# shg8/3DGS.cpp

Hardware: NVIDIA H100
Metric: frames/sec (higher is better)
Workload: dtype f32

## Files before the change

3dgs.cpp_b200/csrc/gsb_api.cu:

```cuda
#include <math.h>
#include <stdio.h>
#include <stdlib.h>
#include <string.h>

#include <algorithm>
#include <new>
#include <thread>
#include <vector>

#include "gsb_ctx.cuh"

using namespace gsb;

namespace {
thread_local std::string g_create_error;
}

namespace gsb {

int fail(gsb_ctx* c, int code, const char* what, cudaError_t e) {
    if (c) {
        c->err = what;
        if (e != cudaSuccess) {
            c->err += ": ";
            c->err += cudaGetErrorString(e);
        }
    }
    return code;
}

void drop_graphs(gsb_ctx* ctx) {
    for (auto& g : ctx->graphs) {
        if (g.exec) cudaGraphExecDestroy(g.exec);
        g = MiddleGraph{};
    }
}

template <typename T>
static int grow_zeroed(gsb_ctx* ctx, DevArray<T>& a, uint64_t count, const char* name) {
    if (count <= a.count) return GSB_OK;
    const char* step = "cudaMalloc";
    cudaError_t e = a.grow(count);
    if (e == cudaSuccess) {
        step = "cudaMemsetAsync";
        e = cudaMemsetAsync(a, 0, count * sizeof(T), ctx->stream);
    }
    if (e == cudaSuccess) {
        step = "cudaStreamSynchronize";
        e = cudaStreamSynchronize(ctx->stream);
    }
    if (e == cudaSuccess) return GSB_OK;
    a.reset();
    return fail(ctx, e == cudaErrorMemoryAllocation ? GSB_ERR_OOM : GSB_ERR_CUDA, (std::string(step) + " of " + name).c_str(), e);
}

int ensure_sort_status(gsb_ctx* ctx, uint64_t items) {
    const uint32_t tiles = (uint32_t)((items + sort_tile_items() - 1) / sort_tile_items());
    if ((uint64_t)tiles * 256 <= ctx->sort_status.count) return GSB_OK;
    ctx->alloc_gen++;
    return grow_zeroed(ctx, ctx->sort_status, (uint64_t)tiles * 256, "ctx->sort_status");
}

int ensure_arena(gsb_ctx* ctx, uint64_t capacity) {
    if (capacity <= ctx->capacity) return GSB_OK;
    if (capacity >= (1ull << 30)) return fail(ctx, GSB_ERR_OVERFLOW, "instance arena limited to 2^30 - 1 entries");
    ctx->capacity = 0;
    ctx->alloc_gen++;
    ctx->frame.recorded = false;
    CK(ctx->keys[0].grow(capacity + 16));
    CK(ctx->keys[1].grow(capacity + 16));
    CK(ctx->vals[0].grow(capacity + 16));
    CK(ctx->vals[1].grow(capacity + 16));
    int rc = ensure_sort_status(ctx, std::max<uint64_t>(capacity, ctx->n));
    if (rc != GSB_OK) return rc;
    ctx->capacity = capacity;
    return GSB_OK;
}

uint32_t bits_for(uint32_t count) {
    uint32_t b = 0;
    while (b < 32 && (1ull << b) < count) b++;
    return b;
}

uint32_t quantise_hint(uint64_t hint) {
    uint64_t q = 4096;
    while (q < hint && q < (1ull << 31)) q <<= 1;
    return (uint32_t)q;
}

size_t bytes_per_pixel(int fmt) { return fmt == GSB_FORMAT_RGBA32F ? 16 : 4; }

static void take_hints(gsb_ctx* ctx) {
    ctx->frame.pending = false;
    ctx->m_hint = ctx->ctl_host->num_instances;
    ctx->nv_hint = ctx->ctl_host->num_visible;
}

int wait_frame(gsb_ctx* ctx) {
    if (ctx->frame.pending) {
        CK(cudaEventSynchronize(ctx->ev_done));
        take_hints(ctx);
    }
    return GSB_OK;
}

void poll_frame(gsb_ctx* ctx) {
    if (ctx->frame.pending && cudaEventQuery(ctx->ev_done) == cudaSuccess) take_hints(ctx);
}

int regrow_after_overflow(gsb_ctx* ctx, cudaStream_t stream) {
    if (!ctx->ctl_host->overflow) return GSB_OK;
    const uint64_t want = ctx->ctl_host->instances_total + ctx->ctl_host->instances_total / 4 + 4096;
    int rc = ensure_arena(ctx, want);
    if (rc != GSB_OK) return rc;
    CK(cudaMemsetAsync(&ctx->ctl->overflow_sticky, 0, sizeof(uint32_t), stream));
    ctx->regrow_count++;
    return GSB_OK;
}

static __global__ void k_frame_init(Control* ctl, uint32_t* __restrict__ project_status, uint32_t project_chunks,
                                    unsigned long long* __restrict__ emit_status, uint32_t emit_chunks, uint2* __restrict__ ranges,
                                    uint32_t num_tiles, uint32_t* __restrict__ route_status, uint32_t route_words) {
    const uint32_t i = blockIdx.x * blockDim.x + threadIdx.x, stride = gridDim.x * blockDim.x;
    uint32_t* w = reinterpret_cast<uint32_t*>(ctl);
    for (uint32_t k = i; k < sizeof(Control) / 4; k += stride) {
        if (k == offsetof(Control, overflow_sticky) / 4) continue;
        if (k == offsetof(Control, epoch) / 4) w[k] += 16u;
        else w[k] = 0u;
    }
    for (uint32_t k = i; k < project_chunks; k += stride) project_status[k] = 0u;
    for (uint32_t k = i; k < emit_chunks; k += stride) emit_status[k] = 0ull;
    for (uint32_t k = i; k < num_tiles; k += stride) ranges[k] = make_uint2(0xffffffffu, 0xffffffffu);
    for (uint32_t k = i; k < route_words; k += stride) route_status[k] = 0u;
}

cudaError_t launch_frame_init(Control* ctl, uint32_t* project_status, uint32_t project_chunks, unsigned long long* emit_status,
                              uint32_t emit_chunks, uint2* ranges, uint32_t num_tiles, cudaStream_t s, uint32_t* route_status,
                              uint32_t route_words) {
    const uint32_t work = std::max<uint32_t>(std::max(std::max(std::max(project_chunks, emit_chunks), num_tiles), route_words),
                                             (uint32_t)(sizeof(Control) / 4));
    const uint32_t blocks = std::min<uint32_t>((work + 255) / 256, 132u * 4u);
    k_frame_init<<<blocks, 256, 0, s>>>(ctl, project_status, project_chunks, emit_status, emit_chunks, ranges, num_tiles, route_status,
                                        route_words);
    return cudaGetLastError();
}

int enqueue_middle(gsb_ctx* ctx, const FramePlan& fp, const Survivors& sv, cudaStream_t stream, bool events) {
    SortParams sa;
    sa.keys[0] = sv.dkeys[0];
    sa.keys[1] = sv.dkeys[1];
    sa.vals[0] = sv.dvals[0];
    sa.vals[1] = sv.dvals[1];
    sa.d_m = &ctx->ctl->num_visible;
    sa.m_hint = fp.nv_q;
    sa.key_bits = 32;
    sa.status = ctx->sort_status;
    sa.status_tiles = (uint32_t)(ctx->sort_status.count / 256);
    sa.d_epoch = &ctx->ctl->epoch;
    sa.sc = &ctx->ctl->sort_depth;
    sa.num_sms = ctx->num_sms;
    sa.discard_sorted_keys = true;
    uint32_t depth_passes = 0;
    CK(launch_sort(sa, &depth_passes, stream));
    const int fin_a = depth_passes & 1;
    if (events) CK(cudaEventRecord(ctx->ev[2], stream));

    EmitParams ep{};
    ep.sorted_cid = sv.dvals[fin_a];
    ep.nv_hint = fp.nv_q;
    ep.tiles_x = fp.bins_x;
    ep.coarse_shift = fp.cs;
    ep.keys = ctx->keys[0];
    ep.vals = ctx->vals[0];
    ep.capacity = (uint32_t)ctx->capacity;
    ep.status = sv.emit_status;
    ep.ctl = ctx->ctl;
    ep.num_sms = ctx->num_sms;
    ep.recs = sv.recs;
    ep.cull = (ctx->tile_cull >= 1 && fp.cs == 0) ? 1 : 0;
    ep.dbg_offsets = ctx->debug ? ctx->dbg_offsets.p : nullptr;
    CK(launch_emit(ep, stream));
    if (events) CK(cudaEventRecord(ctx->ev[3], stream));

    if (ctx->debug) {
        CK(cudaStreamSynchronize(stream));
        uint32_t m = 0;
        CK(cudaMemcpy(&m, &ctx->ctl->num_instances, sizeof m, cudaMemcpyDeviceToHost));
        if (ctx->dbg_keys_unsorted) CK(cudaDeviceSynchronize());
        CK(ctx->dbg_keys_unsorted.grow(m));
        CK(ctx->dbg_vals_unsorted.grow(m));
        CK(cudaMemcpyAsync(ctx->dbg_keys_unsorted, ctx->keys[0], (size_t)m * 4, cudaMemcpyDeviceToDevice, stream));
        CK(cudaMemcpyAsync(ctx->dbg_vals_unsorted, ctx->vals[0], (size_t)m * 4, cudaMemcpyDeviceToDevice, stream));
    }

    SortParams sp;
    sp.keys[0] = ctx->keys[0];
    sp.keys[1] = ctx->keys[1];
    sp.vals[0] = ctx->vals[0];
    sp.vals[1] = ctx->vals[1];
    sp.d_m = &ctx->ctl->num_instances;
    sp.m_hint = fp.m_q;
    sp.key_bits = bits_for(fp.bins);
    sp.status = ctx->sort_status;
    sp.status_tiles = (uint32_t)(ctx->sort_status.count / 256);
    sp.d_epoch = &ctx->ctl->epoch;
    sp.epoch_base = 4;
    sp.sc = &ctx->ctl->sort_tile;
    sp.num_sms = ctx->num_sms;
    sp.events = events ? ctx->ev_sort : nullptr;
    sp.ranges = ctx->ranges;
    sp.discard_sorted_keys = !ctx->debug && fp.cs == 0;
    sp.range_key_mask = fp.cs ? 0xffffu : 0u;
    uint32_t passes = 0;
    CK(launch_sort(sp, &passes, stream));
    if (events) CK(cudaEventRecord(ctx->ev[4], stream));
    if (passes == 0) CK(launch_ranges_single_tile(sp.d_m, ctx->ranges, stream));
    if (events) CK(cudaEventRecord(ctx->ev[5], stream));
    if (depth_passes != fp.depth_passes || passes != fp.passes) return fail(ctx, GSB_ERR_CUDA, "internal: pass count mismatch");
    return GSB_OK;
}

int launch_middle_graph(gsb_ctx* ctx, const FramePlan& fp, const Survivors& sv, cudaStream_t stream) {
    MiddleKey key;
    key.tiles_x = fp.tiles_x;
    key.num_tiles = fp.T;
    key.nv_q = fp.nv_q;
    key.m_q = fp.m_q;
    key.cull = (uint32_t)ctx->tile_cull;
    key.cs = fp.cs;
    key.alloc_gen = ctx->alloc_gen;
    key.sv = sv;
    MiddleGraph* slot = nullptr;
    for (auto& g : ctx->graphs)
        if (g.exec && g.key == key) slot = &g;
    if (!slot) {
        slot = &ctx->graphs[0];
        for (auto& g : ctx->graphs)
            if (!g.exec || (slot->exec && g.last_use < slot->last_use)) slot = &g;
        if (slot->exec) cudaGraphExecDestroy(slot->exec);
        *slot = MiddleGraph{};
        cudaGraph_t graph = nullptr;
        CK(cudaStreamBeginCapture(ctx->stream, cudaStreamCaptureModeThreadLocal));
        int rc = enqueue_middle(ctx, fp, sv, ctx->stream, false);
        cudaError_t e = cudaStreamEndCapture(ctx->stream, &graph);
        if (rc != GSB_OK) {
            if (graph) cudaGraphDestroy(graph);
            return rc;
        }
        if (e != cudaSuccess) return fail(ctx, GSB_ERR_CUDA, "cudaStreamEndCapture", e);
        e = cudaGraphInstantiate(&slot->exec, graph, 0);
        cudaGraphDestroy(graph);
        if (e != cudaSuccess) {
            slot->exec = nullptr;
            return fail(ctx, GSB_ERR_CUDA, "cudaGraphInstantiate", e);
        }
        slot->key = key;
    }
    slot->last_use = ++ctx->graph_clock;
    CK(cudaGraphLaunch(slot->exec, stream));
    return GSB_OK;
}

int ensure_ranges(gsb_ctx* ctx, uint32_t W, uint32_t H) {
    const uint32_t T = ((W + GSB_TILE - 1) / GSB_TILE) * ((H + GSB_TILE - 1) / GSB_TILE);
    if (T > ctx->ranges.count) {
        ctx->alloc_gen++;
        CK(ctx->ranges.grow(T));
    }
    return GSB_OK;
}

int plan_frame(gsb_ctx* ctx, const gsb_uniforms* ubo, uint32_t rb, uint32_t re, cudaStream_t stream, FramePlan* out) {
    FramePlan fp{};
    fp.W = ubo->width;
    fp.H = ubo->height;
    fp.tiles_x = (fp.W + GSB_TILE - 1) / GSB_TILE;
    fp.tiles_y = (fp.H + GSB_TILE - 1) / GSB_TILE;
    fp.T = fp.tiles_x * fp.tiles_y;
    fp.rb = rb;
    fp.re = re;
    {
        int rc = ensure_ranges(ctx, fp.W, fp.H);
        if (rc != GSB_OK) return rc;
    }
    const uint32_t n = (uint32_t)ctx->n;
    fp.nv_q = std::min<uint32_t>(quantise_hint(ctx->nv_hint ? ctx->nv_hint : n), quantise_hint(n));
    fp.m_q = quantise_hint(ctx->m_hint ? ctx->m_hint : std::min<uint64_t>(ctx->capacity, 4u * 1024 * 1024));
    fp.cs = (ctx->tile_cull == 2 && !ctx->debug && !ctx->backward) ? ctx->coarse_shift : 0u;
    fp.bins_x = (fp.tiles_x + (1u << fp.cs) - 1) >> fp.cs;
    fp.bins = fp.bins_x * ((fp.tiles_y + (1u << fp.cs) - 1) >> fp.cs);
    if (fp.cs && fp.bins > 65536u) {
        fp.cs = 0;
        fp.bins_x = fp.tiles_x;
        fp.bins = fp.T;
    }
    fp.depth_passes = 4;
    fp.passes = (bits_for(fp.bins) + 7) / 8;
    fp.fin = (int)(fp.passes & 1);
    if (++ctx->frames_since_epoch_clear >= (1u << 27)) {
        CK(cudaMemsetAsync(ctx->sort_status, 0, ctx->sort_status.count * sizeof(unsigned long long), stream));
        CK(cudaMemsetAsync(&ctx->ctl->epoch, 0, sizeof(uint32_t), stream));
        ctx->frames_since_epoch_clear = 0;
    }
    *out = fp;
    return GSB_OK;
}

ProjectParams project_params(const gsb_ctx* ctx, const gsb_uniforms& ubo, uint32_t rb, uint32_t re) {
    ProjectParams pp{};
    pp.pos_op = ctx->pos_op;
    pp.cov_a = ctx->cov_a;
    pp.cov_b = ctx->cov_b;
    pp.sh = ctx->sh;
    pp.sh_half = ctx->scene_sh_half ? 1 : 0;
    pp.n = (uint32_t)ctx->n;
    pp.ubo = ubo;
    pp.tile_row_begin = rb;
    pp.tile_row_end = re;
    pp.recs = ctx->recs;
    pp.dkeys = ctx->dkeys[0];
    pp.dvals = ctx->dvals[0];
    pp.status = ctx->project_status;
    pp.ctl = ctx->ctl;
    pp.dbg_tiles = ctx->dbg_tiles;
    pp.dbg_aabb = ctx->dbg_aabb;
    return pp;
}

static int enqueue_front(gsb_ctx* ctx, const gsb_uniforms* ubo, uint32_t rb, uint32_t re, const Survivors& sv, cudaStream_t stream,
                         FramePlan* out) {
    FramePlan fp{};
    int rc = plan_frame(ctx, ubo, rb, re, stream, &fp);
    if (rc != GSB_OK) return rc;
    const uint32_t chunks = (uint32_t)((ctx->n + 255) / 256);
    const bool timers = ctx->timers;
    CK(launch_frame_init(ctx->ctl, ctx->project_status, std::max(chunks, 1u), ctx->emit_status, std::max(chunks, 1u), ctx->ranges, fp.T, stream));
    if (timers) CK(cudaEventRecord(ctx->ev[0], stream));

    CK(launch_project(project_params(ctx, *ubo, rb, re), ctx->debug, ctx->antialiased, stream));
    if (timers) CK(cudaEventRecord(ctx->ev[1], stream));

    if (ctx->use_graph && !timers && !ctx->debug) rc = launch_middle_graph(ctx, fp, sv, stream);
    else rc = enqueue_middle(ctx, fp, sv, stream, timers);
    if (rc != GSB_OK) return rc;
    *out = fp;
    return GSB_OK;
}

int enqueue_blend(gsb_ctx* ctx, const FramePlan& fp, const Survivors& sv, uint32_t b0, uint32_t b1, void* band_out, size_t pitch,
                  int fmt, cudaStream_t stream, void* const* peer_frames, int num_peer_frames) {
    BlendParams bp{};
    bp.recs = sv.recs;
    bp.vals = ctx->vals[fp.fin];
    bp.keys = ctx->keys[fp.fin];
    bp.ranges = ctx->ranges;
    bp.width = fp.W;
    bp.height = fp.H;
    bp.tiles_x = fp.tiles_x;
    bp.coarse_shift = fp.cs;
    bp.bins_x = fp.bins_x;
    bp.tile_row_begin = b0;
    bp.tile_row_end = b1;
    bp.out = static_cast<unsigned char*>(band_out) + (size_t)(b0 - fp.rb) * GSB_TILE * pitch;
    bp.out_first_row = b0 * GSB_TILE;
    bp.num_peers = num_peer_frames;
    for (int k = 0; k < num_peer_frames && k < GSB_MAX_SHARDS; k++) bp.peer_frames[k] = peer_frames[k];
    if (num_peer_frames > 0) bp.out_first_row = 0;
    bp.row_pitch_bytes = pitch;
    bp.format = fmt;
    bp.mode = ctx->mode;
    bp.stats = ctx->debug ? 2 : (ctx->timers ? 1 : 0);
    bp.ctl = ctx->ctl;
    bp.record = (ctx->backward && fp.cs == 0 && num_peer_frames == 0) ? ctx->bw_record.p : nullptr;
    for (int c = 0; c < 3; c++) bp.background[c] = ctx->background[c];
    CK(launch_blend(bp, stream));
    return GSB_OK;
}

int enqueue_tail(gsb_ctx* ctx, const FramePlan& fp, const gsb_uniforms& ubo, cudaStream_t stream) {
    if (ctx->timers) CK(cudaEventRecord(ctx->ev[6], stream));
    CK(cudaMemcpyAsync(ctx->ctl_host, ctx->ctl, offsetof(Control, sort_depth), cudaMemcpyDeviceToHost, stream));
    CK(cudaEventRecord(ctx->ev_done, stream));
    LastFrame& f = ctx->frame;
    f.plan = fp;
    f.ubo = ubo;
    f.mode = ctx->mode;
    f.antialiased = ctx->antialiased;
    for (int c = 0; c < 3; c++) f.background[c] = ctx->background[c];
    f.scene_gen = ctx->scene_gen;
    f.pending = true;
    f.exists = true;
    f.debug = ctx->debug;
    f.timers = ctx->timers;
    f.recorded = ctx->backward && fp.cs == 0;
    f.band = !(fp.rb == 0 && fp.re == fp.tiles_y);
    return GSB_OK;
}

static int enqueue_frame(gsb_ctx* ctx, const gsb_uniforms* ubo, uint32_t rb, uint32_t re, void* out_dev, size_t pitch, int fmt,
                  cudaStream_t stream) {
    ctx->frame.recorded = false;
    if (ctx->backward) CK(ctx->bw_record.grow((size_t)ubo->width * ubo->height));
    const Survivors sv{ctx->recs, {ctx->dkeys[0], ctx->dkeys[1]}, {ctx->dvals[0], ctx->dvals[1]}, ctx->emit_status};
    FramePlan fp{};
    int rc = enqueue_front(ctx, ubo, rb, re, sv, stream, &fp);
    if (rc != GSB_OK) return rc;
    rc = enqueue_blend(ctx, fp, sv, rb, re, out_dev, pitch, fmt, stream);
    if (rc != GSB_OK) return rc;
    return enqueue_tail(ctx, fp, *ubo, stream);
}

int check_image(gsb_ctx* ctx, const gsb_uniforms* ubo, int fmt) {
    if (fmt < GSB_FORMAT_RGBA32F || fmt > GSB_FORMAT_BGRA8) return fail(ctx, GSB_ERR_INVALID, "bad format");
    const uint32_t W = ubo->width, H = ubo->height;
    if (W == 0 || H == 0 || W > 16u * 65535u || H > 16u * 65535u) return fail(ctx, GSB_ERR_INVALID, "bad image size");
    return GSB_OK;
}

int check_render_args(gsb_ctx* ctx, const gsb_uniforms* ubo, uint32_t& rb, uint32_t& re, const void* out, size_t& pitch,
                      int fmt) {
    if (!ctx) return GSB_ERR_INVALID;
    if (!ubo || !out) return fail(ctx, GSB_ERR_INVALID, "null argument");
    if (!ctx->pos_op) return fail(ctx, GSB_ERR_NO_SCENE, "no scene uploaded");
    const int rc = check_image(ctx, ubo, fmt);
    if (rc != GSB_OK) return rc;
    const uint32_t W = ubo->width, H = ubo->height;
    const uint32_t tiles_y = (H + GSB_TILE - 1) / GSB_TILE;
    if (re > tiles_y) re = tiles_y;
    if (rb >= re) return fail(ctx, GSB_ERR_INVALID, "empty tile-row band");
    const size_t tight = (size_t)W * bytes_per_pixel(fmt);
    if (pitch == 0) pitch = tight;
    if (pitch < tight || (pitch % (fmt == GSB_FORMAT_RGBA32F ? 16 : 4)) != 0) return fail(ctx, GSB_ERR_INVALID, "bad row pitch");
    return GSB_OK;
}

}

extern "C" {

int gsb_abi_version(void) { return GSB_ABI_VERSION; }

int gsb_device_count(void) {
    int n = 0;
    if (cudaGetDeviceCount(&n) != cudaSuccess) {
        cudaGetLastError();
        return 0;
    }
    return n;
}

const char* gsb_last_error(const gsb_ctx* ctx) { return ctx ? ctx->err.c_str() : g_create_error.c_str(); }

int gsb_create(int device, gsb_ctx** out) {
    if (!out) return GSB_ERR_INVALID;
    *out = nullptr;
    int count = 0;
    cudaError_t e = cudaGetDeviceCount(&count);
    if (e != cudaSuccess || count <= 0 || device < 0 || device >= count) {
        cudaGetLastError();
        g_create_error = "no usable CUDA device (libgsb200 has no CPU path)";
        if (e != cudaSuccess) g_create_error += std::string(": ") + cudaGetErrorString(e);
        return GSB_ERR_NO_DEVICE;
    }
    gsb_ctx* ctx = new (std::nothrow) gsb_ctx();
    if (!ctx) return GSB_ERR_OOM;
    ctx->device = device;
    auto bail = [&](const char* what, cudaError_t err) {
        g_create_error = std::string(what) + ": " + cudaGetErrorString(err);
        gsb_destroy(ctx);
        return GSB_ERR_CUDA;
    };
    if ((e = cudaSetDevice(device)) != cudaSuccess) return bail("cudaSetDevice", e);
    cudaDeviceProp prop;
    if ((e = cudaGetDeviceProperties(&prop, device)) != cudaSuccess) return bail("cudaGetDeviceProperties", e);
    cudaFuncAttributes fa;
    if (prop.major != 9 || prop.minor != 0 || cudaFuncGetAttributes(&fa, k_frame_init) != cudaSuccess) {
        cudaGetLastError();
        g_create_error = "libgsb200 is built for sm_90a (H100, compute capability 9.0) only; device is sm_" +
                         std::to_string(prop.major) + std::to_string(prop.minor);
        gsb_destroy(ctx);
        return GSB_ERR_NO_DEVICE;
    }
    ctx->num_sms = prop.multiProcessorCount;
    if (const char* v = getenv("GSB_HOST_DIRECT")) ctx->host_direct = atoi(v) != 0;
    if (const char* v = getenv("GSB_COARSE_SHIFT")) ctx->coarse_shift = (uint32_t)std::min(2, std::max(1, atoi(v)));
    if ((e = sort_prepare()) != cudaSuccess) return bail("sort_prepare", e);
    if ((e = cudaStreamCreateWithFlags(&ctx->stream, cudaStreamNonBlocking)) != cudaSuccess) return bail("cudaStreamCreate", e);
    if ((e = dev_alloc(&ctx->ctl, 1)) != cudaSuccess) return bail("cudaMalloc", e);
    if ((e = cudaMemset(ctx->ctl, 0, sizeof(Control))) != cudaSuccess) return bail("cudaMemset", e);
    if ((e = cudaDeviceSynchronize()) != cudaSuccess) return bail("cudaDeviceSynchronize", e);
    if ((e = cudaMallocHost(reinterpret_cast<void**>(&ctx->ctl_host), sizeof(Control))) != cudaSuccess) return bail("cudaMallocHost", e);
    memset(ctx->ctl_host, 0, sizeof(Control));
    for (auto& ev : ctx->ev)
        if ((e = cudaEventCreate(&ev)) != cudaSuccess) return bail("cudaEventCreate", e);
    for (auto& ev : ctx->ev_sort)
        if ((e = cudaEventCreate(&ev)) != cudaSuccess) return bail("cudaEventCreate", e);
    if ((e = cudaEventCreateWithFlags(&ctx->ev_done, cudaEventDisableTiming)) != cudaSuccess) return bail("cudaEventCreate", e);
    *out = ctx;
    return GSB_OK;
}

void gsb_destroy(gsb_ctx* ctx) {
    if (!ctx) return;
    cudaSetDevice(ctx->device);
    if (ctx->stream) cudaStreamSynchronize(ctx->stream);
    cudaDeviceSynchronize();
    drop_graphs(ctx);
    shard_destroy(ctx);
    if (ctx->ctl) cudaFree(ctx->ctl);
    if (ctx->ctl_host) cudaFreeHost(ctx->ctl_host);
    for (auto& ev : ctx->ev)
        if (ev) cudaEventDestroy(ev);
    for (auto& ev : ctx->ev_sort)
        if (ev) cudaEventDestroy(ev);
    if (ctx->ev_done) cudaEventDestroy(ctx->ev_done);
    if (ctx->stream) cudaStreamDestroy(ctx->stream);
    delete ctx;
}

int gsb_scene_upload(gsb_ctx* ctx, const float* vertices, uint64_t n, gsb_memory mem) {
    if (!ctx) return GSB_ERR_INVALID;
    if (n && !vertices) return fail(ctx, GSB_ERR_INVALID, "null vertices");
    if (n >= (1ull << 30)) return fail(ctx, GSB_ERR_INVALID, "scene limited to 2^30 - 1 Gaussians");
    CK(cudaSetDevice(ctx->device));
    CK(cudaStreamSynchronize(ctx->stream));
    if (ctx->pos_op) CK(cudaDeviceSynchronize());
    ctx->frame.pending = ctx->frame.exists = false;
    ctx->n = 0;
    ctx->alloc_gen++;
    ctx->scene_gen++;
    drop_graphs(ctx);
    CK(ctx->pos_op.grow(n));
    CK(ctx->cov_a.grow(n));
    CK(ctx->cov_b.grow(n));
    ctx->scene_sh_half = ctx->sh_half;
    CK(ctx->sh.grow(n * (ctx->scene_sh_half ? 24 : 48)));
    CK(ctx->recs.grow(n * GSB_REC_F4));
    CK(ctx->dkeys[0].grow(n));
    CK(ctx->dkeys[1].grow(n));
    CK(ctx->dvals[0].grow(n));
    CK(ctx->dvals[1].grow(n));
    CK(ctx->project_status.grow((n + 255) / 256));
    CK(ctx->emit_status.grow((n + 255) / 256));
    if (ctx->debug) {
        CK(ctx->dbg_tiles.grow(n));
        CK(ctx->dbg_aabb.grow(n));
        CK(ctx->dbg_offsets.grow(n));
    }
    if (mem == GSB_MEM_DEVICE) {
        const uint64_t chunk = std::min<uint64_t>(std::max<uint64_t>(n, 1), 1u << 20);
        for (uint64_t off = 0; off < n; off += chunk) {
            const uint64_t cnt = std::min(chunk, n - off);
            cudaError_t e = launch_cov3d(vertices + off * 60, cnt, off, ctx->pos_op, ctx->cov_a, ctx->cov_b, ctx->sh, 1.0f, ctx->stream, ctx->scene_sh_half);
            if (e != cudaSuccess) return fail(ctx, GSB_ERR_CUDA, "cov3d precompute", e);
        }
        CK(cudaStreamSynchronize(ctx->stream));
    } else if (n) {
        cudaPointerAttributes pa{};
        const bool caller_pinned = cudaPointerGetAttributes(&pa, vertices) == cudaSuccess && pa.type == cudaMemoryTypeHost;
        cudaGetLastError();
        const uint64_t chunk = std::min<uint64_t>(n, 1u << 18);
        float* dev_stage[2] = {nullptr, nullptr};
        float* pin_stage[2] = {nullptr, nullptr};
        cudaEvent_t slot_free[2] = {nullptr, nullptr};
        cudaError_t e = cudaSuccess;
        for (int k = 0; k < 2 && e == cudaSuccess; k++) {
            e = dev_alloc(&dev_stage[k], chunk * 60);
            if (e == cudaSuccess && !caller_pinned) e = cudaMallocHost(reinterpret_cast<void**>(&pin_stage[k]), chunk * 60 * sizeof(float));
            if (e == cudaSuccess) e = cudaEventCreateWithFlags(&slot_free[k], cudaEventDisableTiming);
        }
        const unsigned hw = std::max(1u, std::min(std::thread::hardware_concurrency(), 8u));
        uint64_t idx = 0;
        for (uint64_t off = 0; off < n && e == cudaSuccess; off += chunk, idx++) {
            const int k = (int)(idx & 1);
            const uint64_t cnt = std::min(chunk, n - off);
            const float* src = vertices + off * 60;
            if (idx >= 2) e = cudaEventSynchronize(slot_free[k]);
            if (e != cudaSuccess) break;
            if (!caller_pinned) {
                const size_t bytes = cnt * 60 * sizeof(float);
                const unsigned nt = bytes >= (8u << 20) ? hw : 1u;
                std::vector<std::thread> pool;
                const size_t per = (bytes / nt + 63) & ~size_t(63);
                for (unsigned t = 1; t < nt; t++) {
                    const size_t b = std::min(bytes, t * per), en = std::min(bytes, b + per);
                    if (b < en) pool.emplace_back([=] { memcpy(reinterpret_cast<char*>(pin_stage[k]) + b, reinterpret_cast<const char*>(src) + b, en - b); });
                }
                memcpy(pin_stage[k], src, std::min(bytes, per));
                for (auto& th : pool) th.join();
                src = pin_stage[k];
            }
            e = cudaMemcpyAsync(dev_stage[k], src, cnt * 60 * sizeof(float), cudaMemcpyHostToDevice, ctx->stream);
            if (e == cudaSuccess) e = launch_cov3d(dev_stage[k], cnt, off, ctx->pos_op, ctx->cov_a, ctx->cov_b, ctx->sh, 1.0f, ctx->stream, ctx->scene_sh_half);
            if (e == cudaSuccess) e = cudaEventRecord(slot_free[k], ctx->stream);
        }
        if (e == cudaSuccess) e = cudaStreamSynchronize(ctx->stream);
        else cudaStreamSynchronize(ctx->stream);
        for (int k = 0; k < 2; k++) {
            if (dev_stage[k]) cudaFree(dev_stage[k]);
            if (pin_stage[k]) cudaFreeHost(pin_stage[k]);
            if (slot_free[k]) cudaEventDestroy(slot_free[k]);
        }
        if (e != cudaSuccess) return fail(ctx, e == cudaErrorMemoryAllocation ? GSB_ERR_OOM : GSB_ERR_CUDA, "scene upload", e);
    }
    ctx->n = n;
    ctx->m_hint = 0;
    ctx->nv_hint = 0;
    {
        int rc = ensure_sort_status(ctx, std::max<uint64_t>(n, ctx->capacity));
        if (rc != GSB_OK) return rc;
    }
    if (ctx->capacity == 0) {
        int rc = ensure_arena(ctx, std::max<uint64_t>(n, 1024));
        if (rc != GSB_OK) return rc;
    }
    return GSB_OK;
}

uint64_t gsb_scene_size(const gsb_ctx* ctx) { return ctx ? ctx->n : 0; }

int gsb_set_mode(gsb_ctx* ctx, gsb_mode mode) {
    if (!ctx || (mode != GSB_MODE_EXACT && mode != GSB_MODE_FAST)) return GSB_ERR_INVALID;
    ctx->mode = mode;
    return GSB_OK;
}

int gsb_set_sh_storage(gsb_ctx* ctx, int half_precision) {
    if (!ctx) return GSB_ERR_INVALID;
    ctx->sh_half = half_precision != 0;
    return GSB_OK;
}

int gsb_set_debug(gsb_ctx* ctx, int debug) {
    if (!ctx) return GSB_ERR_INVALID;
    CK(cudaSetDevice(ctx->device));
    ctx->debug = debug != 0;
    if (ctx->debug && ctx->n) {
        CK(ctx->dbg_tiles.grow(ctx->n));
        CK(ctx->dbg_aabb.grow(ctx->n));
        CK(ctx->dbg_offsets.grow(ctx->n));
    }
    return GSB_OK;
}

int gsb_set_graph(gsb_ctx* ctx, int enabled) {
    if (!ctx) return GSB_ERR_INVALID;
    ctx->use_graph = enabled != 0;
    return GSB_OK;
}

int gsb_host_alloc(void** out, size_t bytes) {
    if (!out) return GSB_ERR_INVALID;
    *out = nullptr;
    cudaError_t e = cudaMallocHost(out, bytes ? bytes : 1);
    if (e != cudaSuccess) {
        cudaGetLastError();
        g_create_error = std::string("cudaMallocHost: ") + cudaGetErrorString(e);
        return e == cudaErrorMemoryAllocation ? GSB_ERR_OOM : GSB_ERR_CUDA;
    }
    return GSB_OK;
}

void gsb_host_free(void* p) {
    if (p) cudaFreeHost(p);
}

int gsb_set_tile_cull(gsb_ctx* ctx, int level) {
    if (!ctx || level < 0 || level > 2) return GSB_ERR_INVALID;
    ctx->tile_cull = level;
    return GSB_OK;
}

int gsb_set_timers(gsb_ctx* ctx, int enabled) {
    if (!ctx) return GSB_ERR_INVALID;
    ctx->timers = enabled != 0;
    return GSB_OK;
}

int gsb_reserve_instances(gsb_ctx* ctx, uint64_t capacity) {
    if (!ctx) return GSB_ERR_INVALID;
    CK(cudaSetDevice(ctx->device));
    int rc = wait_frame(ctx);
    if (rc != GSB_OK) return rc;
    return ensure_arena(ctx, capacity);
}

int gsb_render_async(gsb_ctx* ctx, const gsb_uniforms* ubo, uint32_t rb, uint32_t re, void* out_device, size_t pitch,
                     gsb_format fmt, void* stream) {
    int rc = check_render_args(ctx, ubo, rb, re, out_device, pitch, fmt);
    if (rc != GSB_OK) return rc;
    CK(cudaSetDevice(ctx->device));
    poll_frame(ctx);
    return enqueue_frame(ctx, ubo, rb, re, out_device, pitch, fmt, stream_or_own(ctx, stream));
}

int gsb_render(gsb_ctx* ctx, const gsb_uniforms* ubo, uint32_t rb, uint32_t re, void* out, size_t pitch, gsb_memory out_mem,
               gsb_format fmt, void* stream) {
    int rc = check_render_args(ctx, ubo, rb, re, out, pitch, fmt);
    if (rc != GSB_OK) return rc;
    CK(cudaSetDevice(ctx->device));
    cudaStream_t s = stream_or_own(ctx, stream);
    const uint32_t H = ubo->height;
    const uint32_t rows = std::min(H, re * GSB_TILE) - rb * GSB_TILE;
    const size_t tight = (size_t)ubo->width * bytes_per_pixel(fmt);

    void* dev_out = out;
    size_t dev_pitch = pitch;
    bool staged = false;
    if (out_mem == GSB_MEM_HOST) {
        cudaPointerAttributes pa{};
        const bool pinned = ctx->host_direct && cudaPointerGetAttributes(&pa, out) == cudaSuccess &&
                            pa.type == cudaMemoryTypeHost && pa.devicePointer != nullptr;
        cudaGetLastError();
        if (pinned) {
            dev_out = pa.devicePointer;
        } else {
            CK(ctx->fb.grow(tight * rows));
            dev_out = ctx->fb;
            dev_pitch = tight;
            staged = true;
        }
    }
    for (int attempt = 0;; attempt++) {
        rc = enqueue_frame(ctx, ubo, rb, re, dev_out, dev_pitch, fmt, s);
        if (rc != GSB_OK) return rc;
        rc = wait_frame(ctx);
        if (rc != GSB_OK) return rc;
        if (!ctx->ctl_host->overflow) break;
        if (attempt >= 3) return fail(ctx, GSB_ERR_OVERFLOW, "instance arena overflow persists after regrow");
        rc = regrow_after_overflow(ctx, s);
        if (rc != GSB_OK) return rc;
    }
    if (staged) {
        CK(cudaMemcpy2DAsync(out, pitch, dev_out, dev_pitch, tight, rows, cudaMemcpyDeviceToHost, s));
        CK(cudaStreamSynchronize(s));
    }
    return GSB_OK;
}

int gsb_get_stats(gsb_ctx* ctx, gsb_stats* out) {
    if (!ctx || !out) return GSB_ERR_INVALID;
    memset(out, 0, sizeof *out);
    if (!ctx->frame.exists) return fail(ctx, GSB_ERR_INVALID, "no frame rendered yet");
    CK(cudaSetDevice(ctx->device));
    const int rc = wait_frame(ctx);
    if (rc != GSB_OK) return rc;
    const Control* c = ctx->ctl_host;
    out->num_gaussians = ctx->n;
    out->num_visible = c->num_visible;
    out->num_instances = c->instances_total;
    out->num_instances_aabb = c->candidates_total;
    out->blend_consumed = c->blend_consumed;
    out->blend_warp_visits = c->blend_walked;
    out->blend_pixel_hits = c->blend_hits;
    out->blend_staged = c->blend_staged;
    out->instance_capacity = ctx->capacity;
    out->sort_passes = ctx->frame.plan.passes;
    out->sort_depth_passes = ctx->frame.plan.depth_passes;
    out->regrow_count = ctx->regrow_count;
    if (ctx->frame.timers) {
        float ms = 0.f;
        CK(cudaEventElapsedTime(&ms, ctx->ev[0], ctx->ev[1]));
        out->preprocess_ms = ms;
        CK(cudaEventElapsedTime(&ms, ctx->ev[1], ctx->ev[2]));
        out->sort_depth_ms = ms;
        CK(cudaEventElapsedTime(&ms, ctx->ev[2], ctx->ev[3]));
        out->preprocess_sort_ms = ms;
        CK(cudaEventElapsedTime(&ms, ctx->ev[3], ctx->ev[4]));
        out->sort_tile_ms = ms;
        out->sort_ms = out->sort_depth_ms + out->sort_tile_ms;
        if (ctx->frame.plan.passes) {
            CK(cudaEventElapsedTime(&ms, ctx->ev[3], ctx->ev_sort[0]));
            out->sort_hist_ms = ms;
            for (uint32_t p = 0; p < ctx->frame.plan.passes && p < 8; p++) {
                CK(cudaEventElapsedTime(&ms, ctx->ev_sort[p], ctx->ev_sort[p + 1]));
                out->sort_pass_ms[p] = ms;
            }
        }
        CK(cudaEventElapsedTime(&ms, ctx->ev[4], ctx->ev[5]));
        out->tile_boundary_ms = ms;
        CK(cudaEventElapsedTime(&ms, ctx->ev[5], ctx->ev[6]));
        out->render_ms = ms;
        CK(cudaEventElapsedTime(&ms, ctx->ev[0], ctx->ev[6]));
        out->frame_ms = ms;
        if (ctx->shard) {
            CK(cudaEventElapsedTime(&ms, ctx->ev[5], ctx->ev[7]));
            out->shard_blend_ms = ms;
            CK(cudaEventElapsedTime(&ms, ctx->ev[7], ctx->ev[6]));
            out->shard_wait_ms = ms;
        }
    }
    if (c->overflow || c->overflow_sticky) {
        CK(cudaMemsetAsync(&ctx->ctl->overflow_sticky, 0, sizeof(uint32_t), ctx->stream));
        CK(cudaStreamSynchronize(ctx->stream));
        ctx->ctl_host->overflow_sticky = 0;
        return fail(ctx, GSB_ERR_OVERFLOW, c->overflow ? "last frame overflowed the instance arena (gsb_render regrows; gsb_render_async does not)"
                                                       : "an earlier gsb_render_async frame overflowed the instance arena (its image is incomplete)");
    }
    return GSB_OK;
}

int gsb_set_backward(gsb_ctx* ctx, int enabled) {
    if (!ctx) return GSB_ERR_INVALID;
    if (ctx->shard) return fail(ctx, GSB_ERR_INVALID, "gsb_set_backward: sharded contexts have no backward pass");
    CK(cudaSetDevice(ctx->device));
    ctx->backward = enabled != 0;
    if (!ctx->backward) {
        CK(cudaStreamSynchronize(ctx->stream));
        ctx->bw_record.reset();
        ctx->frame.recorded = false;
        ctx->bw_det = {};
    }
    return GSB_OK;
}

int gsb_set_antialiased(gsb_ctx* ctx, int enabled) {
    if (!ctx) return GSB_ERR_INVALID;
    if (ctx->shard) return fail(ctx, GSB_ERR_INVALID, "gsb_set_antialiased: sharded contexts have no anti-aliased mode");
    ctx->antialiased = enabled != 0;
    return GSB_OK;
}

int gsb_set_background(gsb_ctx* ctx, const float* rgb) {
    if (!ctx) return GSB_ERR_INVALID;
    const float v[3] = {rgb ? rgb[0] : 0.0f, rgb ? rgb[1] : 0.0f, rgb ? rgb[2] : 0.0f};
    for (float x : v)
        if (!isfinite(x)) return fail(ctx, GSB_ERR_INVALID, "gsb_set_background: the colour must be finite");
    for (int c = 0; c < 3; c++) ctx->background[c] = v[c];
    return GSB_OK;
}

int gsb_set_backward_deterministic(gsb_ctx* ctx, int enabled) {
    if (!ctx) return GSB_ERR_INVALID;
    if (ctx->shard) return fail(ctx, GSB_ERR_INVALID, "gsb_set_backward_deterministic: sharded contexts have no backward pass");
    ctx->bw_deterministic = enabled != 0;
    return GSB_OK;
}

static int ensure_det_buffers(gsb_ctx* ctx, uint64_t n) {
    DetBuffers& d = ctx->bw_det;
    const uint64_t cap = ctx->capacity;
    CK(d.slots.grow(cap * 11));
    CK(d.keys[0].grow(cap));
    CK(d.keys[1].grow(cap));
    CK(d.pos[0].grow(cap));
    CK(d.pos[1].grow(cap));
    const uint32_t tiles = (uint32_t)((cap + sort_tile_items() - 1) / sort_tile_items());
    CK(d.status.grow((uint64_t)std::max<uint32_t>(tiles, 1) * 256));
    CK(d.sc.grow(1));
    if (n > d.runs.count) CK(d.runs.grow(n));
    return GSB_OK;
}

static int check_recorded_frame(gsb_ctx* ctx, int no_frame, const char* fn) {
    const LastFrame& f = ctx->frame;
    auto bad = [&](int code, const char* what) { return fail(ctx, code, (std::string(fn) + ": " + what).c_str()); };
    if (f.scene_gen == 0) return bad(no_frame, "no frame rendered yet");
    if (f.scene_gen != ctx->scene_gen) return bad(GSB_ERR_INVALID, "the scene was uploaded or stepped after the last frame");
    if (!f.recorded) return bad(GSB_ERR_INVALID, "the last frame was rendered with gsb_set_backward off, or the arena grew since");
    if (f.band) return bad(GSB_ERR_INVALID, "the last frame was a band of tile rows, not the whole frame");
    const int rc = wait_frame(ctx);
    if (rc != GSB_OK) return rc;
    if (ctx->ctl_host->overflow) return bad(GSB_ERR_INVALID, "the last frame overflowed the instance arena (its lists are incomplete)");
    return GSB_OK;
}

static int render_backward(gsb_ctx* ctx, const char* fn, bool args_ok, const float* vertices, const float* grad_image, size_t pitch,
                           float* grad_vertices, gsb_uniforms* grad_ubo, float* density, void* stream) {
    if (!ctx) return GSB_ERR_INVALID;
    auto msg = [&](const char* what) { return std::string(fn) + ": " + what; };
    if (ctx->shard) return fail(ctx, GSB_ERR_INVALID, msg("sharded contexts have no backward pass").c_str());
    if (!ctx->pos_op) return fail(ctx, GSB_ERR_NO_SCENE, msg("no scene uploaded").c_str());
    CK(cudaSetDevice(ctx->device));
    int rc = check_recorded_frame(ctx, GSB_ERR_NO_SCENE, fn);
    if (rc != GSB_OK) return rc;
    if (ctx->scene_sh_half) return fail(ctx, GSB_ERR_INVALID, msg("fp16 SH storage has no backward pass").c_str());
    if (!args_ok) return fail(ctx, GSB_ERR_INVALID, msg("null argument").c_str());
    const LastFrame& f = ctx->frame;
    const size_t tight = (size_t)f.ubo.width * sizeof(float4);
    if (pitch == 0) pitch = tight;
    if (pitch < tight || pitch % sizeof(float4) != 0) return fail(ctx, GSB_ERR_INVALID, msg("bad row pitch").c_str());
    const uint64_t n = ctx->n;
    rc = grow_zeroed(ctx, ctx->bw_scratch, n * 9, "ctx->bw_scratch");
    if (rc != GSB_OK) return rc;
    if (density) {
        rc = grow_zeroed(ctx, ctx->bw_abs, n * 2, "ctx->bw_abs");
        if (rc != GSB_OK) return rc;
    }
    if (grad_ubo)
        CK(ctx->bw_cam_partials.grow((uint64_t)ctx->num_sms * 4 * GSB_UBO_WORDS));
    const bool det = ctx->bw_deterministic;
    if (det) {
        rc = ensure_det_buffers(ctx, n);
        if (rc != GSB_OK) return rc;
    }
    cudaStream_t s = stream_or_own(ctx, stream);
    if (grad_vertices) CK(cudaMemsetAsync(grad_vertices, 0, (size_t)n * 60 * sizeof(float), s));
    if (n == 0) {
        if (grad_ubo) CK(cudaMemsetAsync(grad_ubo, 0, sizeof(gsb_uniforms), s));
        return GSB_OK;
    }
    BackwardParams bp{};
    bp.recs = ctx->recs;
    bp.vals = ctx->vals[f.plan.fin];
    bp.ranges = ctx->ranges;
    bp.record = ctx->bw_record;
    bp.ctl = ctx->ctl;
    bp.width = f.ubo.width;
    bp.height = f.ubo.height;
    bp.tiles_x = f.plan.tiles_x;
    bp.num_tiles = f.plan.T;
    bp.mode = f.mode;
    bp.ubo = f.ubo;
    bp.vertices = vertices;
    bp.cov_a = ctx->cov_a;
    bp.cov_b = ctx->cov_b;
    bp.grad_image = grad_image;
    bp.row_pitch_bytes = pitch;
    bp.scratch = ctx->bw_scratch;
    bp.grad_vertices = grad_vertices;
    bp.num_sms = ctx->num_sms;
    bp.cam_partials = grad_ubo ? ctx->bw_cam_partials.p : nullptr;
    bp.grad_ubo = grad_ubo;
    bp.abs_scratch = density ? ctx->bw_abs.p : nullptr;
    bp.density = density;
    const float3 bg = make_float3(f.background[0], f.background[1], f.background[2]);
    if (!det) {
        CK(launch_backward(bp, f.antialiased, bg, s));
        return GSB_OK;
    }
    const DetBuffers& d = ctx->bw_det;
    bp.det_slots = d.slots;
    DetBackward db{};
    db.keys[0] = d.keys[0];
    db.keys[1] = d.keys[1];
    db.pos[0] = d.pos[0];
    db.pos[1] = d.pos[1];
    db.runs = d.runs;
    db.sc = d.sc;
    db.status = d.status;
    db.status_tiles = (uint32_t)(d.status.count / 256);
    db.m_hint = quantise_hint(ctx->m_hint);
    db.key_bits = std::max<uint32_t>(bits_for((uint32_t)n), 1u);
    CK(launch_backward(bp, f.antialiased, bg, s, &db));
    return GSB_OK;
}

int gsb_render_backward(gsb_ctx* ctx, const float* vertices, const float* grad_image, size_t pitch, float* grad_vertices, void* stream) {
    return render_backward(ctx, "gsb_render_backward", vertices && grad_image && grad_vertices, vertices, grad_image, pitch, grad_vertices,
                           nullptr, nullptr, stream);
}

int gsb_render_backward_camera(gsb_ctx* ctx, const float* vertices, const float* grad_image, size_t pitch, float* grad_vertices,
                               gsb_uniforms* grad_uniforms, void* stream) {
    return render_backward(ctx, "gsb_render_backward_camera", vertices && grad_image && grad_uniforms, vertices, grad_image, pitch,
                           grad_vertices, grad_uniforms, nullptr, stream);
}

int gsb_render_backward_density(gsb_ctx* ctx, const float* vertices, const float* grad_image, size_t pitch, float* grad_vertices,
                                gsb_uniforms* grad_uniforms, float* density, void* stream) {
    return render_backward(ctx, "gsb_render_backward_density", vertices && grad_image && density && (grad_vertices || grad_uniforms),
                           vertices, grad_image, pitch, grad_vertices, grad_uniforms, density, stream);
}

int gsb_background_gradient(gsb_ctx* ctx, const float* grad_image, size_t pitch, float* grad_background, void* stream) {
    if (!ctx) return GSB_ERR_INVALID;
    const char* fn = "gsb_background_gradient";
    auto msg = [&](const char* what) { return std::string(fn) + ": " + what; };
    if (ctx->shard) return fail(ctx, GSB_ERR_INVALID, msg("sharded contexts have no backward pass").c_str());
    if (!ctx->pos_op) return fail(ctx, GSB_ERR_NO_SCENE, msg("no scene uploaded").c_str());
    CK(cudaSetDevice(ctx->device));
    const int rc = check_recorded_frame(ctx, GSB_ERR_NO_SCENE, fn);
    if (rc != GSB_OK) return rc;
    if (!grad_image || !grad_background) return fail(ctx, GSB_ERR_INVALID, msg("null argument").c_str());
    const LastFrame& f = ctx->frame;
    const size_t tight = (size_t)f.ubo.width * sizeof(float4);
    if (pitch == 0) pitch = tight;
    if (pitch < tight || pitch % sizeof(float4) != 0) return fail(ctx, GSB_ERR_INVALID, msg("bad row pitch").c_str());
    CK(ctx->bg_partials.grow((uint64_t)background_grad_rows(f.ubo.height) * 3));
    CK(launch_background_grad(ctx->bw_record, grad_image, pitch, f.ubo.width, f.ubo.height, ctx->bg_partials, grad_background,
                              stream_or_own(ctx, stream)));
    return GSB_OK;
}

int gsb_adam_step(gsb_ctx* ctx, float* params, float* exp_avg, float* exp_avg_sq, const float* grad_vertices, float* vertices,
                  const gsb_adam_config* cfg, void* stream) {
    if (!ctx) return GSB_ERR_INVALID;
    auto bad = [&](const char* what) { return fail(ctx, GSB_ERR_INVALID, (std::string("gsb_adam_step: ") + what).c_str()); };
    if (ctx->shard) return bad("sharded contexts have no training step");
    if (!ctx->pos_op) return fail(ctx, GSB_ERR_NO_SCENE, "gsb_adam_step: no scene uploaded");
    if (ctx->scene_sh_half) return bad("fp16 SH storage has no training step");
    if (!params || !exp_avg || !exp_avg_sq || !grad_vertices || !vertices || !cfg) return bad("null argument");
    for (const void* p : {(const void*)params, (const void*)exp_avg, (const void*)exp_avg_sq, (const void*)grad_vertices, (const void*)vertices})
        if (reinterpret_cast<uintptr_t>(p) % 16) return bad("array not aligned to 16 B");
    for (float lr : cfg->lr)
        if (!(lr >= 0.0f)) return bad("learning rate below 0 or NaN");
    if (!(cfg->beta1 >= 0.0f && cfg->beta1 < 1.0f) || !(cfg->beta2 >= 0.0f && cfg->beta2 < 1.0f)) return bad("beta outside [0, 1)");
    if (!(cfg->eps >= 0.0f)) return bad("eps below 0 or NaN");
    if (!(cfg->bias_correction1 > 0.0f && cfg->bias_correction1 <= 1.0f) ||
        !(cfg->bias_correction2_sqrt > 0.0f && cfg->bias_correction2_sqrt <= 1.0f))
        return bad("bias correction outside (0, 1]");
    if (cfg->selective > 1) return bad("selective is neither 0 nor 1");
    CK(cudaSetDevice(ctx->device));
    if (cfg->selective) {
        const int rc = check_recorded_frame(ctx, GSB_ERR_INVALID, "gsb_adam_step: selective");
        if (rc != GSB_OK) return rc;
    }
    AdamParams P{};
    P.params = reinterpret_cast<float4*>(params);
    P.exp_avg = reinterpret_cast<float4*>(exp_avg);
    P.exp_avg_sq = reinterpret_cast<float4*>(exp_avg_sq);
    P.grad = reinterpret_cast<const float4*>(grad_vertices);
    P.vertices = reinterpret_cast<float4*>(vertices);
    P.pos_op = ctx->pos_op;
    P.cov_a = ctx->cov_a;
    P.cov_b = ctx->cov_b;
    P.sh = reinterpret_cast<float4*>(ctx->sh.p);
    P.n = ctx->n;
    P.recs = cfg->selective ? ctx->recs.p : nullptr;
    P.ctl = ctx->ctl;
    for (int g = 0; g < 6; g++) P.lr[g] = cfg->lr[g];
    P.beta1 = cfg->beta1;
    P.beta2 = cfg->beta2;
    P.eps = cfg->eps;
    P.bias_correction1 = cfg->bias_correction1;
    P.bias_correction2_sqrt = cfg->bias_correction2_sqrt;
    cudaStream_t s = stream_or_own(ctx, stream);
    ctx->scene_gen++;
    CK(launch_adam(P, ctx->num_sms, s));
    return GSB_OK;
}

size_t gsb_debug_size(gsb_ctx* ctx, gsb_buffer which) {
    if (!ctx) return 0;
    const uint64_t n = ctx->n;
    if (which == GSB_BUF_COV3D) return (size_t)n * 6 * sizeof(float);
    if (!ctx->frame.exists || !ctx->debug || !ctx->frame.debug) return 0;
    if (wait_frame(ctx) != GSB_OK) return 0;
    const uint64_t m = ctx->ctl_host->num_instances;
    switch (which) {
        case GSB_BUF_ATTR: return (size_t)n * sizeof(gsb_vertex_attribute);
        case GSB_BUF_TILES_OVERLAP:
        case GSB_BUF_PREFIX_SUM: return (size_t)n * 4;
        case GSB_BUF_KEYS_UNSORTED:
        case GSB_BUF_KEYS_SORTED: return (size_t)m * 8;
        case GSB_BUF_VALS_UNSORTED:
        case GSB_BUF_VALS_SORTED: return (size_t)m * 4;
        case GSB_BUF_TILE_BOUNDARY: return (size_t)ctx->frame.plan.T * 8;
        case GSB_BUF_DEPTH_ORDER: return (size_t)ctx->ctl_host->num_visible * 4;
        case GSB_BUF_EMIT_OFFSETS: return (size_t)ctx->ctl_host->num_visible * 8;
        default: return 0;
    }
}

int gsb_debug_download(gsb_ctx* ctx, gsb_buffer which, void* dst, size_t bytes) {
    if (!ctx || !dst) return GSB_ERR_INVALID;
    CK(cudaSetDevice(ctx->device));
    const size_t need = gsb_debug_size(ctx, which);
    if (need == 0 && which != GSB_BUF_COV3D) return fail(ctx, GSB_ERR_INVALID, "debug buffer unavailable (enable gsb_set_debug before rendering)");
    if (bytes < need) return fail(ctx, GSB_ERR_INVALID, "destination too small");
    CK(cudaStreamSynchronize(ctx->stream));
    CK(cudaDeviceSynchronize());
    const uint64_t n = ctx->n;
    const uint32_t nv = ctx->frame.exists ? ctx->ctl_host->num_visible : 0;
    const uint64_t m = ctx->frame.exists ? ctx->ctl_host->num_instances : 0;
    switch (which) {
        case GSB_BUF_COV3D: {
            std::vector<float4> a(n);
            std::vector<float2> b(n);
            if (n) {
                CK(cudaMemcpy(a.data(), ctx->cov_a, n * sizeof(float4), cudaMemcpyDeviceToHost));
                CK(cudaMemcpy(b.data(), ctx->cov_b, n * sizeof(float2), cudaMemcpyDeviceToHost));
            }
            float* o = static_cast<float*>(dst);
            for (uint64_t i = 0; i < n; i++) {
                o[i * 6 + 0] = a[i].x;
                o[i * 6 + 1] = a[i].y;
                o[i * 6 + 2] = a[i].z;
                o[i * 6 + 3] = a[i].w;
                o[i * 6 + 4] = b[i].x;
                o[i * 6 + 5] = b[i].y;
            }
            return GSB_OK;
        }
        case GSB_BUF_ATTR: {
            std::vector<float4> recs((size_t)nv * GSB_REC_F4);
            std::vector<uint4> aabb(n);
            if (nv) CK(cudaMemcpy(recs.data(), ctx->recs, recs.size() * sizeof(float4), cudaMemcpyDeviceToHost));
            if (n) CK(cudaMemcpy(aabb.data(), ctx->dbg_aabb, n * sizeof(uint4), cudaMemcpyDeviceToHost));
            gsb_vertex_attribute* o = static_cast<gsb_vertex_attribute*>(dst);
            memset(o, 0, n * sizeof(gsb_vertex_attribute));
            for (uint32_t c = 0; c < nv; c++) {
                const float4 r0 = recs[(size_t)c * GSB_REC_F4], r1 = recs[(size_t)c * GSB_REC_F4 + 1], r2 = recs[(size_t)c * GSB_REC_F4 + 2],
                             r3 = recs[(size_t)c * GSB_REC_F4 + 3];
                uint32_t i;
                memcpy(&i, &r3.y, 4);
                if (i >= n) return fail(ctx, GSB_ERR_CUDA, "corrupt compact record");
                gsb_vertex_attribute& a = o[i];
                a.conic_opacity[0] = r0.z;
                a.conic_opacity[1] = r0.w;
                a.conic_opacity[2] = r1.x;
                a.conic_opacity[3] = r1.y;
                a.color_radii[0] = r2.x;
                a.color_radii[1] = r2.y;
                a.color_radii[2] = r2.z;
                a.color_radii[3] = r3.x;
                a.aabb[0] = aabb[i].x;
                a.aabb[1] = aabb[i].y;
                a.aabb[2] = aabb[i].z;
                a.aabb[3] = aabb[i].w;
                a.uv[0] = r0.x;
                a.uv[1] = r0.y;
                a.depth = r2.w;
                a.magic = 0x4d415449u;
            }
            return GSB_OK;
        }
        case GSB_BUF_TILES_OVERLAP:
            if (n) CK(cudaMemcpy(dst, ctx->dbg_tiles, n * 4, cudaMemcpyDeviceToHost));
            return GSB_OK;
        case GSB_BUF_PREFIX_SUM: {
            uint32_t* o = static_cast<uint32_t*>(dst);
            if (n) CK(cudaMemcpy(o, ctx->dbg_tiles, n * 4, cudaMemcpyDeviceToHost));
            uint32_t run = 0;
            for (uint64_t i = 0; i < n; i++) {
                run += o[i];
                o[i] = run;
            }
            return GSB_OK;
        }
        case GSB_BUF_KEYS_UNSORTED:
        case GSB_BUF_KEYS_SORTED:
        case GSB_BUF_VALS_UNSORTED:
        case GSB_BUF_VALS_SORTED: {
            const bool sorted = which == GSB_BUF_KEYS_SORTED || which == GSB_BUF_VALS_SORTED;
            const bool want_keys = which == GSB_BUF_KEYS_UNSORTED || which == GSB_BUF_KEYS_SORTED;
            std::vector<float4> recs((size_t)nv * GSB_REC_F4);
            if (nv) CK(cudaMemcpy(recs.data(), ctx->recs, recs.size() * sizeof(float4), cudaMemcpyDeviceToHost));
            std::vector<uint32_t> tk(m), cv(m);
            const uint32_t* ksrc = sorted ? ctx->keys[ctx->frame.plan.fin] : ctx->dbg_keys_unsorted;
            const uint32_t* vsrc = sorted ? ctx->vals[ctx->frame.plan.fin] : ctx->dbg_vals_unsorted;
            if (m) {
                CK(cudaMemcpy(tk.data(), ksrc, m * 4, cudaMemcpyDeviceToHost));
                CK(cudaMemcpy(cv.data(), vsrc, m * 4, cudaMemcpyDeviceToHost));
            }
            for (uint64_t k = 0; k < m; k++) {
                if (cv[k] >= nv) return fail(ctx, GSB_ERR_CUDA, "corrupt payload");
                const float4 r2 = recs[(size_t)cv[k] * GSB_REC_F4 + 2], r3 = recs[(size_t)cv[k] * GSB_REC_F4 + 3];
                uint32_t depth_bits, orig;
                memcpy(&depth_bits, &r2.w, 4);
                memcpy(&orig, &r3.y, 4);
                if (want_keys) static_cast<uint64_t*>(dst)[k] = ((uint64_t)tk[k] << 32) | depth_bits;
                else static_cast<uint32_t*>(dst)[k] = orig;
            }
            return GSB_OK;
        }
        case GSB_BUF_DEPTH_ORDER: {
            std::vector<float4> recs((size_t)nv * GSB_REC_F4);
            std::vector<uint32_t> cid(nv);
            if (nv) {
                CK(cudaMemcpy(recs.data(), ctx->recs, recs.size() * sizeof(float4), cudaMemcpyDeviceToHost));
                CK(cudaMemcpy(cid.data(), ctx->dvals[ctx->frame.plan.depth_passes & 1], (size_t)nv * 4, cudaMemcpyDeviceToHost));
            }
            for (uint32_t j = 0; j < nv; j++) {
                if (cid[j] >= nv) return fail(ctx, GSB_ERR_CUDA, "corrupt depth order");
                memcpy(static_cast<uint32_t*>(dst) + j, &recs[(size_t)cid[j] * GSB_REC_F4 + 3].y, 4);
            }
            return GSB_OK;
        }
        case GSB_BUF_EMIT_OFFSETS:
            if (nv) CK(cudaMemcpy(dst, ctx->dbg_offsets, (size_t)nv * 8, cudaMemcpyDeviceToHost));
            return GSB_OK;
        case GSB_BUF_TILE_BOUNDARY: {
            CK(cudaMemcpy(dst, ctx->ranges, need, cudaMemcpyDeviceToHost));
            uint32_t* o = static_cast<uint32_t*>(dst);
            for (size_t t = 0; t < need / 8; t++) {
                if (o[2 * t] == 0xffffffffu) o[2 * t] = o[2 * t + 1] = 0u;
                else o[2 * t + 1] = ~o[2 * t + 1];
            }
            return GSB_OK;
        }
        default: return fail(ctx, GSB_ERR_INVALID, "unknown buffer id");
    }
}

static int sort_pairs_impl(gsb_ctx* ctx, void* keys, uint32_t* vals, void* keys_tmp, uint32_t* vals_tmp, uint64_t m,
                           uint32_t key_bits, int key_bytes, void* stream, const char* what) {
    if (!ctx) return GSB_ERR_INVALID;
    if (m == 0) return GSB_OK;
    if (!keys || !vals || !keys_tmp || !vals_tmp || key_bits == 0 || key_bits > 8u * (uint32_t)key_bytes) return fail(ctx, GSB_ERR_INVALID, "bad argument");
    if (m >= (1ull << 30)) return fail(ctx, GSB_ERR_INVALID, "sort limited to 2^30 - 1 pairs");
    CK(cudaSetDevice(ctx->device));
    cudaStream_t s = stream_or_own(ctx, stream);
    const uint32_t tiles = (uint32_t)((m + sort_tile_items() - 1) / sort_tile_items());
    const size_t status_bytes = (size_t)tiles * 256 * 8;
    unsigned char* scratch = nullptr;
    CK(dev_alloc(&scratch, status_bytes + sizeof(SortCtl) + 4));
    unsigned long long* status = reinterpret_cast<unsigned long long*>(scratch);
    SortCtl* sc = reinterpret_cast<SortCtl*>(scratch + status_bytes);
    uint32_t* d_m = reinterpret_cast<uint32_t*>(sc + 1);
    cudaError_t e = cudaMemsetAsync(scratch, 0, status_bytes + sizeof(SortCtl), s);
    const uint32_t m32 = (uint32_t)m;
    if (e == cudaSuccess) e = cudaMemcpyAsync(d_m, &m32, 4, cudaMemcpyHostToDevice, s);
    SortParams sp;
    sp.keys[0] = keys;
    sp.keys[1] = keys_tmp;
    sp.key_bytes = key_bytes;
    sp.vals[0] = vals;
    sp.vals[1] = vals_tmp;
    sp.d_m = d_m;
    sp.m_hint = m32;
    sp.key_bits = key_bits;
    sp.status = status;
    sp.status_tiles = tiles;
    sp.epoch_base = 8;
    sp.sc = sc;
    sp.num_sms = ctx->num_sms;
    uint32_t passes = 0;
    if (e == cudaSuccess) e = launch_sort(sp, &passes, s);
    if (e == cudaSuccess && (passes & 1)) {
        e = cudaMemcpyAsync(keys, keys_tmp, m * (size_t)key_bytes, cudaMemcpyDeviceToDevice, s);
        if (e == cudaSuccess) e = cudaMemcpyAsync(vals, vals_tmp, m * 4, cudaMemcpyDeviceToDevice, s);
    }
    if (e == cudaSuccess) e = cudaStreamSynchronize(s);
    cudaFree(scratch);
    if (e != cudaSuccess) return fail(ctx, GSB_ERR_CUDA, what, e);
    return GSB_OK;
}

int gsb_sort_pairs(gsb_ctx* ctx, uint64_t* keys, uint32_t* vals, uint64_t* keys_tmp, uint32_t* vals_tmp, uint64_t m,
                   uint32_t key_bits, void* stream) {
    return sort_pairs_impl(ctx, keys, vals, keys_tmp, vals_tmp, m, key_bits, 8, stream, "gsb_sort_pairs");
}

int gsb_sort_pairs32(gsb_ctx* ctx, uint32_t* keys, uint32_t* vals, uint32_t* keys_tmp, uint32_t* vals_tmp, uint64_t m,
                     uint32_t key_bits, void* stream) {
    return sort_pairs_impl(ctx, keys, vals, keys_tmp, vals_tmp, m, key_bits, 4, stream, "gsb_sort_pairs32");
}

}
```

3dgs.cpp_b200/csrc/gsb_backward.cu:

```cuda
#include <algorithm>
#include <type_traits>

#include "gsb_cull.cuh"
#include "gsb_exp.cuh"
#include "gsb_geom.cuh"
#include "gsb_internal.cuh"

namespace gsb {

namespace {

constexpr unsigned FULL = 0xffffffffu;
constexpr int BW_THREADS = 256;
constexpr int BW_BATCH = 256;
constexpr int BW_NACC = 9;
constexpr int BW_NABS = 2;
constexpr int BW_DET_BATCH = 128;
constexpr int BW_WARPS = BW_THREADS / 32;
template <bool DET>
constexpr uint32_t bw_batch = DET ? BW_DET_BATCH : BW_BATCH;
constexpr int PB_THREADS = 256;

struct __align__(16) BwRec {
    float4 q0;
    float4 q1;
    float4 q2;
};

__device__ __forceinline__ float* det_partials() {
    extern __shared__ float s_dyn[];
    return s_dyn;
}

struct BackwardBgParams : BackwardParams {
    float3 bg;
};
template <bool BG>
using BwParams = std::conditional_t<BG, BackwardBgParams, BackwardParams>;
template <bool BG>
BwParams<BG> bw_params(const BackwardParams& p, float3 bg) {
    if constexpr (BG) return BackwardBgParams{p, bg};
    else return p;
}

template <int MODE, bool ABSGRAD, bool DET = false, bool BG = false>
__global__ void __launch_bounds__(BW_THREADS) k_blend_backward(const __grid_constant__ BwParams<BG> P) {
    constexpr int NACC = BW_NACC + (ABSGRAD ? BW_NABS : 0);
    __shared__ BwRec s_rec[bw_batch<DET>];
    __shared__ double s_acc[DET ? 1 : BW_BATCH][NACC];
    __shared__ uint32_t s_max;

    const int tid = threadIdx.x, lane = tid & 31, warp = tid >> 5;
    const uint32_t tile = blockIdx.x;
    const uint32_t tx = tile % P.tiles_x, ty = tile / P.tiles_x;
    uint2 range = P.ranges[tile];
    range.y = ~range.y;
    const uint32_t px = tx * GSB_TILE + (warp & 1) * 8 + (lane & 7);
    const uint32_t py = ty * GSB_TILE + (warp >> 1) * 4 + (lane >> 3);
    const bool inside = px < P.width && py < P.height;
    const float fx = (float)px, fy = (float)py;

    float T = 1.0f, gr = 0.f, gg = 0.f, gb = 0.f;
    uint32_t last = 0;
    if (inside) {
        const uint2 r = P.record[(size_t)py * P.width + px];
        T = __uint_as_float(r.x);
        last = r.y;
        const float4 g = *reinterpret_cast<const float4*>(reinterpret_cast<const unsigned char*>(P.grad_image) + (size_t)py * P.row_pitch_bytes +
                                                          (size_t)px * sizeof(float4));
        gr = g.x, gg = g.y, gb = g.z;
    }
    if (tid == 0) s_max = 0;
    __syncthreads();
    const uint32_t wmax = __reduce_max_sync(FULL, last);
    if (lane == 0 && wmax) atomicMax(&s_max, wmax);
    __syncthreads();
    const uint32_t max_last = s_max;
    if (range.x >= range.y) return;

    float acc_r = 0.f, acc_g = 0.f, acc_b = 0.f;
    if constexpr (BG) {
        acc_r = P.bg.x;
        acc_g = P.bg.y;
        acc_b = P.bg.z;
    }
    for (uint32_t hi = max_last; hi > 0;) {
        const uint32_t lo = hi > bw_batch<DET> ? hi - bw_batch<DET> : 0u;
        const uint32_t cnt = hi - lo;
        __syncthreads();
        if ((uint32_t)tid < cnt) {
            const uint32_t cid = __ldg(P.vals + range.x + lo + (uint32_t)tid);
            const float4* rec = P.recs + (size_t)cid * GSB_REC_F4;
            const float4 a = __ldg(rec), col = __ldg(rec + 2);
            const float2 b = __ldg(reinterpret_cast<const float2*>(rec + 1));
            s_rec[tid].q0 = make_float4(a.x, a.y, -0.5f * a.z, -a.w);
            s_rec[tid].q1 = make_float4(-0.5f * b.x, b.y, col.x, col.y);
            s_rec[tid].q2 = make_float4(col.z, power_cut(b.y), __uint_as_float(cid), 0.f);
            if constexpr (!DET) {
#pragma unroll
                for (int k = 0; k < NACC; k++) s_acc[tid][k] = 0.0;
            }
        }
        __syncthreads();
        for (int k = (int)cnt - 1; k >= 0; k--) {
            const uint32_t pos = lo + (uint32_t)k + 1u;
            const float4 q0 = s_rec[k].q0, q1 = s_rec[k].q1, q2 = s_rec[k].q2;
            const float dx = q0.x - fx, dy = q0.y - fy;
            float pw, e;
            if (MODE == GSB_MODE_EXACT) {
                pw = ((q0.z * dx) * dx + (q1.x * dy) * dy) + (q0.w * dx) * dy;
                e = exp_shared_inrange(pw);
            } else {
                pw = fmaf(q0.z * dx, dx, fmaf(q1.x * dy, dy, (q0.w * dx) * dy));
                e = __expf(pw);
            }
            const float raw = q1.y * e;
            const float al = fminf(0.99f, raw);
            const bool contrib = pos <= last && !(pw > 0.0f || pw < q2.y) && !(al < 1.0f / 255.0f);
            if (!__any_sync(FULL, contrib)) {
                if constexpr (DET) {
                    if (lane == 0) {
#pragma unroll
                        for (int j = 0; j < NACC; j++) det_partials()[(warp * NACC + j) * bw_batch<true> + k] = 0.f;
                    }
                }
                continue;
            }
            float v[BW_NACC];
#pragma unroll
            for (int j = 0; j < BW_NACC; j++) v[j] = 0.f;
            if (contrib) {
                T = T / (1.0f - al);
                const float w = al * T;
                v[6] = gr * w;
                v[7] = gg * w;
                v[8] = gb * w;
                const float dal = T * ((gr * (q1.z - acc_r) + gg * (q1.w - acc_g)) + gb * (q2.x - acc_b));
                acc_r = q1.z * al + (1.0f - al) * acc_r;
                acc_g = q1.w * al + (1.0f - al) * acc_g;
                acc_b = q2.x * al + (1.0f - al) * acc_b;
                if (!(raw > 0.99f)) {
                    const float dpw = dal * raw;
                    v[5] = dal * e;
                    v[0] = dpw * (2.0f * q0.z * dx + q0.w * dy);
                    v[1] = dpw * (2.0f * q1.x * dy + q0.w * dx);
                    v[2] = dpw * (-0.5f * dx * dx);
                    v[3] = dpw * (-dx * dy);
                    v[4] = dpw * (-0.5f * dy * dy);
                }
            }
            float va[BW_NABS];
            if constexpr (ABSGRAD) {
                va[0] = fabsf(v[0]);
                va[1] = fabsf(v[1]);
            }
#pragma unroll
            for (int j = 0; j < BW_NACC; j++) {
#pragma unroll
                for (int o = 16; o > 0; o >>= 1) v[j] += __shfl_xor_sync(FULL, v[j], o);
            }
            if constexpr (ABSGRAD) {
#pragma unroll
                for (int j = 0; j < BW_NABS; j++) {
#pragma unroll
                    for (int o = 16; o > 0; o >>= 1) va[j] += __shfl_xor_sync(FULL, va[j], o);
                }
            }
            if constexpr (DET) {
                if (lane == 0) {
#pragma unroll
                    for (int j = 0; j < BW_NACC; j++) det_partials()[(warp * NACC + j) * bw_batch<true> + k] = v[j];
                    if constexpr (ABSGRAD) {
#pragma unroll
                        for (int j = 0; j < BW_NABS; j++) det_partials()[(warp * NACC + BW_NACC + j) * bw_batch<true> + k] = va[j];
                    }
                }
            } else if (lane == 0) {
#pragma unroll
                for (int j = 0; j < BW_NACC; j++)
                    if (v[j] != 0.f) atomicAdd(&s_acc[k][j], (double)v[j]);
                if constexpr (ABSGRAD) {
#pragma unroll
                    for (int j = 0; j < BW_NABS; j++)
                        if (va[j] != 0.f) atomicAdd(&s_acc[k][BW_NACC + j], (double)va[j]);
                }
            }
        }
        __syncthreads();
        if constexpr (DET) {
            if ((uint32_t)tid < cnt) {
                double* dst = P.det_slots + (size_t)(range.x + lo + (uint32_t)tid) * NACC;
#pragma unroll
                for (int j = 0; j < NACC; j++) {
                    double a = 0.0;
#pragma unroll
                    for (int w = 0; w < BW_WARPS; w++) a += (double)det_partials()[(w * NACC + j) * bw_batch<true> + tid];
                    dst[j] = a;
                }
            }
        } else if ((uint32_t)tid < cnt) {
            double* dst = P.scratch + (size_t)__float_as_uint(s_rec[tid].q2.z) * BW_NACC;
#pragma unroll
            for (int j = 0; j < BW_NACC; j++) {
                const double a = s_acc[tid][j];
                if (a != 0.0) atomicAdd(dst + j, a);
            }
            if constexpr (ABSGRAD) {
                double* dabs = P.abs_scratch + (size_t)__float_as_uint(s_rec[tid].q2.z) * BW_NABS;
#pragma unroll
                for (int j = 0; j < BW_NABS; j++) {
                    const double a = s_acc[tid][BW_NACC + j];
                    if (a != 0.0) atomicAdd(dabs + j, a);
                }
            }
        }
        hi = lo;
    }
    if constexpr (DET) {
        const uint32_t len = range.y - range.x;
        for (uint32_t p = max_last + (uint32_t)tid; p < len; p += BW_THREADS) {
            double* dst = P.det_slots + (size_t)(range.x + p) * NACC;
#pragma unroll
            for (int j = 0; j < NACC; j++) dst[j] = 0.0;
        }
    }
}

__global__ void __launch_bounds__(PB_THREADS) k_density_accumulate(const __grid_constant__ BackwardParams P) {
    const uint32_t nv = P.ctl->num_visible;
    const double hw = 0.5 * (double)P.width, hh = 0.5 * (double)P.height;
    for (uint32_t cid = blockIdx.x * blockDim.x + threadIdx.x; cid < nv; cid += gridDim.x * blockDim.x) {
        const double* sc = P.scratch + (size_t)cid * BW_NACC;
        double* ab = P.abs_scratch + (size_t)cid * BW_NABS;
        const double gx = sc[0] * hw, gy = sc[1] * hh;
        const double ax = ab[0] * hw, ay = ab[1] * hh;
        ab[0] = 0.0;
        ab[1] = 0.0;
        const float4 r3 = __ldg(P.recs + (size_t)cid * GSB_REC_F4 + 3);
        float* d = P.density + (size_t)__float_as_uint(r3.y) * 4;
        d[0] += (float)sqrt(gx * gx + gy * gy);
        d[1] += (float)sqrt(ax * ax + ay * ay);
        d[2] += 1.0f;
        d[3] = fmaxf(d[3], r3.x);
    }
}

__global__ void __launch_bounds__(PB_THREADS) k_det_prepare(const uint32_t* __restrict__ vals, const Control* ctl, uint32_t* __restrict__ keys,
                                                            uint32_t* __restrict__ pos, uint2* __restrict__ runs) {
    const uint32_t m = ctl->num_instances, nv = ctl->num_visible;
    const uint32_t i0 = blockIdx.x * blockDim.x + threadIdx.x, stride = gridDim.x * blockDim.x;
    for (uint32_t p = i0; p < m; p += stride) {
        keys[p] = __ldg(vals + p);
        pos[p] = p;
    }
    for (uint32_t c = i0; c < nv; c += stride) runs[c] = make_uint2(0xffffffffu, 0xffffffffu);
}

template <bool ABSGRAD>
__global__ void __launch_bounds__(PB_THREADS) k_det_reduce(const __grid_constant__ BackwardParams P, const uint32_t* __restrict__ pos,
                                                           const uint2* __restrict__ runs) {
    constexpr int NACC = BW_NACC + (ABSGRAD ? BW_NABS : 0);
    constexpr uint32_t UNROLL = 4;
    const uint32_t nv = P.ctl->num_visible;
    const double* __restrict__ slots = P.det_slots;
    for (uint32_t cid = blockIdx.x * blockDim.x + threadIdx.x; cid < nv; cid += gridDim.x * blockDim.x) {
        double s[NACC];
#pragma unroll
        for (int k = 0; k < NACC; k++) s[k] = 0.0;
        const uint2 r = __ldg(runs + cid);
        if (r.x != 0xffffffffu) {
            const uint32_t end = ~r.y;
            uint32_t j = r.x;
            for (; j + UNROLL <= end; j += UNROLL) {
                double x[UNROLL][NACC];
#pragma unroll
                for (uint32_t u = 0; u < UNROLL; u++) {
                    const double* sl = slots + (size_t)__ldg(pos + j + u) * NACC;
#pragma unroll
                    for (int k = 0; k < NACC; k++) x[u][k] = __ldg(sl + k);
                }
#pragma unroll
                for (uint32_t u = 0; u < UNROLL; u++)
#pragma unroll
                    for (int k = 0; k < NACC; k++) s[k] += x[u][k];
            }
            for (; j < end; j++) {
                const double* sl = slots + (size_t)__ldg(pos + j) * NACC;
#pragma unroll
                for (int k = 0; k < NACC; k++) s[k] += __ldg(sl + k);
            }
        }
        double* sc = P.scratch + (size_t)cid * BW_NACC;
#pragma unroll
        for (int k = 0; k < BW_NACC; k++) sc[k] = s[k];
        if constexpr (ABSGRAD) {
            double* ab = P.abs_scratch + (size_t)cid * BW_NABS;
#pragma unroll
            for (int k = 0; k < BW_NABS; k++) ab[k] = s[BW_NACC + k];
        }
    }
}

constexpr int U_CAMPOS = 0, U_PROJ = 4, U_VIEW = 20, U_TANX = 38, U_TANY = 39;
__host__ __device__ constexpr bool cam_word_live(int j) {
    return j < 3 || (j >= U_PROJ && j < U_VIEW && (j & 3) != 2) || (j >= U_VIEW && j < 36 && (j & 3) != 3) || j >= U_TANX;
}

template <bool CAMERA, bool AA>
__global__ void __launch_bounds__(PB_THREADS) k_preprocess_backward(const __grid_constant__ BackwardParams P) {
    const uint32_t nv = P.ctl->num_visible;
    const gsb_uniforms& U = P.ubo;
    const float* pm = U.proj_mat;
    const float* vm = U.view_mat;
    const bool store_v = !CAMERA || P.grad_vertices != nullptr;
    float cam[GSB_UBO_WORDS];
    if constexpr (CAMERA) {
#pragma unroll
        for (int j = 0; j < GSB_UBO_WORDS; j++) cam[j] = 0.f;
    }
    for (uint32_t cid = blockIdx.x * blockDim.x + threadIdx.x; cid < nv; cid += gridDim.x * blockDim.x) {
        double* sc = P.scratch + (size_t)cid * BW_NACC;
        float d[BW_NACC];
        bool any = false;
#pragma unroll
        for (int k = 0; k < BW_NACC; k++) {
            const double a = sc[k];
            d[k] = (float)a;
            any |= a != 0.0;
        }
        if (!any) continue;
#pragma unroll
        for (int k = 0; k < BW_NACC; k++) sc[k] = 0.0;
        const float4 r2 = __ldg(P.recs + (size_t)cid * GSB_REC_F4 + 2), r3 = __ldg(P.recs + (size_t)cid * GSB_REC_F4 + 3);
        const uint32_t i = __float_as_uint(r3.y);
        const float* v = P.vertices + (size_t)i * 60;
        float* gv = P.grad_vertices + (size_t)i * 60;
        const float px = v[0], py = v[1], pz = v[2];

        const ClipView cv = clip_view(U, px, py, pz);
        const float p_w = cv.p_w, ndcx = cv.ndcx, ndcy = cv.ndcy, vz = cv.vz;
        const Jacobian J = jacobian(U, cv.vx, cv.vy, vz);
        const float limx = J.limx, limy = J.limy, txtz = J.txtz, tytz = J.tytz, tx = J.tx, ty = J.ty;
        const float focal_x = J.focal_x, focal_y = J.focal_y, ja = J.ja, jb = J.jb, g0 = J.g0, g1 = J.g1;
        const float(&T0)[3] = J.T0, (&T1)[3] = J.T1;
        const Cov2d cov = cov2d(T0, T1, __ldg(P.cov_a + i), __ldg(P.cov_b + i));
        const float(&ST0)[3] = cov.tm0, (&ST1)[3] = cov.tm1;
        const float a = cov.m00, b = cov.m10, c = cov.m11;
        const float det = a * c - b * b;

        const float ood = 1.0f / det;
        const float k00 = c * ood, k01 = -b * ood, k11 = a * ood;
        const float dA = d[2], dB = d[3], dC = d[4];
        float da = -((k00 * k00 * dA + k00 * k01 * dB) + k01 * k01 * dC);
        float db = -((2.0f * k00 * k01 * dA + (k00 * k11 + k01 * k01) * dB) + 2.0f * k01 * k11 * dC);
        float dc = -((k01 * k01 * dA + k01 * k11 * dB) + k11 * k11 * dC);
        float comp = 1.0f;
        if constexpr (AA) {
            const float det_f = a * c - cov.m10 * cov.m01, det0 = aa_det0(cov);
            comp = aa_compensation(det0, det_f);
            if (comp > 0.0f) {
                const float h = 0.5f * (d[5] * v[7]) * comp;
                const float gdet0 = h / det0, gdet = -h / det_f;
                da += gdet0 * cov.c11 + gdet * c;
                dc += gdet0 * cov.c00 + gdet * a;
                db -= 2.0f * b * (gdet0 + gdet);
            }
        }
        float G[3][3];
#pragma unroll
        for (int j = 0; j < 3; j++)
#pragma unroll
            for (int k = 0; k < 3; k++) G[j][k] = (da * T0[j] * T0[k] + dc * T1[j] * T1[k]) + 0.5f * db * (T0[j] * T1[k] + T1[j] * T0[k]);
        float dT0[3], dT1[3];
#pragma unroll
        for (int j = 0; j < 3; j++) {
            dT0[j] = 2.0f * da * ST0[j] + db * ST1[j];
            dT1[j] = 2.0f * dc * ST1[j] + db * ST0[j];
        }
        float dja = 0.f, dg0 = 0.f, djb = 0.f, dg1 = 0.f;
#pragma unroll
        for (int r = 0; r < 3; r++) {
            dja += dT0[r] * vm[r * 4 + 0];
            dg0 += dT0[r] * vm[r * 4 + 2];
            djb += dT1[r] * vm[r * 4 + 1];
            dg1 += dT1[r] * vm[r * 4 + 2];
        }
        float dvx = 0.f, dvy = 0.f, dvz = -(ja / vz) * dja - (jb / vz) * djb;
        const float dtx = -(focal_x / (vz * vz)) * dg0, dty = -(focal_y / (vz * vz)) * dg1;
        dvz += -(2.0f * g0 / vz) * dg0 - (2.0f * g1 / vz) * dg1;
        if (txtz < -limx || txtz > limx) dvz += (txtz > 0.0f ? limx : -limx) * dtx;
        else dvx += dtx;
        if (tytz < -limy || tytz > limy) dvz += (tytz > 0.0f ? limy : -limy) * dty;
        else dvy += dty;
        const float dndcx = d[0] * (0.5f * (float)U.width), dndcy = d[1] * (0.5f * (float)U.height);
        const float dhx = dndcx * p_w, dhy = dndcy * p_w, dhw = -(dndcx * ndcx + dndcy * ndcy) * p_w;
        float dp[3];
#pragma unroll
        for (int k = 0; k < 3; k++)
            dp[k] = ((pm[k * 4 + 0] * dhx + pm[k * 4 + 1] * dhy) + pm[k * 4 + 3] * dhw) + ((vm[k * 4 + 0] * dvx + vm[k * 4 + 1] * dvy) + vm[k * 4 + 2] * dvz);

        const float dcr = r2.x > 0.0f ? d[6] : 0.0f;
        const float dcg = d[7], dcb = d[8];
        float x, y, z;
        const float len = view_direction(U.camera_position, px, py, pz, x, y, z);
        const float xx = x * x, yy = y * y, zz = z * z;
        const float basis[16] = {SH_C0,
                                 -SH_C1 * y,
                                 SH_C1 * z,
                                 -SH_C1 * x,
                                 SH_C2_0 * x * y,
                                 SH_C2_1 * y * z,
                                 SH_C2_2 * ((2.0f * zz - xx) - yy),
                                 SH_C2_3 * z * x,
                                 SH_C2_4 * (xx - yy),
                                 SH_C3_0 * (3.0f * xx - yy) * y,
                                 SH_C3_1 * x * y * z,
                                 SH_C3_2 * ((4.0f * zz - xx) - yy) * y,
                                 SH_C3_3 * z * ((2.0f * zz - 3.0f * xx) - 3.0f * yy),
                                 SH_C3_4 * x * ((4.0f * zz - xx) - yy),
                                 SH_C3_5 * (xx - yy) * z,
                                 SH_C3_6 * x * (xx - 3.0f * yy)};
        const float* sh = v + 12;
        float vk[16];
#pragma unroll
        for (int k = 0; k < 16; k++) {
            if (store_v) {
                gv[12 + 3 * k + 0] = basis[k] * dcr;
                gv[12 + 3 * k + 1] = basis[k] * dcg;
                gv[12 + 3 * k + 2] = basis[k] * dcb;
            }
            vk[k] = (sh[3 * k] * dcr + sh[3 * k + 1] * dcg) + sh[3 * k + 2] * dcb;
        }
        const float ddx = -SH_C1 * vk[3] + SH_C2_0 * y * vk[4] - 2.0f * SH_C2_2 * x * vk[6] + SH_C2_3 * z * vk[7] + 2.0f * SH_C2_4 * x * vk[8] +
                          6.0f * SH_C3_0 * x * y * vk[9] + SH_C3_1 * y * z * vk[10] - 2.0f * SH_C3_2 * x * y * vk[11] -
                          6.0f * SH_C3_3 * x * z * vk[12] + SH_C3_4 * ((4.0f * zz - 3.0f * xx) - yy) * vk[13] + 2.0f * SH_C3_5 * x * z * vk[14] +
                          3.0f * SH_C3_6 * (xx - yy) * vk[15];
        const float ddy = -SH_C1 * vk[1] + SH_C2_0 * x * vk[4] + SH_C2_1 * z * vk[5] - 2.0f * SH_C2_2 * y * vk[6] - 2.0f * SH_C2_4 * y * vk[8] +
                          3.0f * SH_C3_0 * (xx - yy) * vk[9] + SH_C3_1 * x * z * vk[10] + SH_C3_2 * ((4.0f * zz - xx) - 3.0f * yy) * vk[11] -
                          6.0f * SH_C3_3 * y * z * vk[12] - 2.0f * SH_C3_4 * x * y * vk[13] - 2.0f * SH_C3_5 * y * z * vk[14] -
                          6.0f * SH_C3_6 * x * y * vk[15];
        const float ddz = SH_C1 * vk[2] + SH_C2_1 * y * vk[5] + 4.0f * SH_C2_2 * z * vk[6] + SH_C2_3 * x * vk[7] + SH_C3_1 * x * y * vk[10] +
                          8.0f * SH_C3_2 * y * z * vk[11] + SH_C3_3 * ((6.0f * zz - 3.0f * xx) - 3.0f * yy) * vk[12] + 8.0f * SH_C3_4 * x * z * vk[13] +
                          SH_C3_5 * (xx - yy) * vk[14];
        const float dot = (x * ddx + y * ddy) + z * ddz;
        dp[0] += (ddx - x * dot) / len;
        dp[1] += (ddy - y * dot) / len;
        dp[2] += (ddz - z * dot) / len;

        if constexpr (CAMERA) {
            const float p3[3] = {px, py, pz}, dv[3] = {dvx, dvy, dvz}, dh[4] = {dhx, dhy, 0.f, dhw};
#pragma unroll
            for (int r = 0; r < 3; r++) {
#pragma unroll
                for (int c = 0; c < 3; c++) cam[U_VIEW + c * 4 + r] += dv[r] * p3[c];
                cam[U_VIEW + 12 + r] += dv[r];
                cam[U_VIEW + r * 4 + 0] += dT0[r] * ja;
                cam[U_VIEW + r * 4 + 1] += dT1[r] * jb;
                cam[U_VIEW + r * 4 + 2] += dT0[r] * g0 + dT1[r] * g1;
            }
#pragma unroll
            for (int k = 0; k < 4; k++) {
                if (k == 2) continue;
#pragma unroll
                for (int c = 0; c < 3; c++) cam[U_PROJ + c * 4 + k] += dh[k] * p3[c];
                cam[U_PROJ + 12 + k] += dh[k];
            }
            cam[U_CAMPOS + 0] -= (ddx - x * dot) / len;
            cam[U_CAMPOS + 1] -= (ddy - y * dot) / len;
            cam[U_CAMPOS + 2] -= (ddz - z * dot) / len;
            const float dfx = dja / vz - (tx / (vz * vz)) * dg0, dfy = djb / vz - (ty / (vz * vz)) * dg1;
            float dtfx = -(focal_x / U.tan_fovx) * dfx, dtfy = -(focal_y / U.tan_fovy) * dfy;
            if (txtz < -limx || txtz > limx) dtfx += (txtz > 0.0f ? 1.3f : -1.3f) * vz * dtx;
            if (tytz < -limy || tytz > limy) dtfy += (tytz > 0.0f ? 1.3f : -1.3f) * vz * dty;
            cam[U_TANX] += dtfx;
            cam[U_TANY] += dtfy;
        }
        if (!store_v) continue;

        const float s[3] = {v[4], v[5], v[6]};
        const float qw = v[8], qx = v[9], qy = v[10], qz = v[11];
        float R[3][3];
        rotation_from_quaternion(qw, qx, qy, qz, R);
        float ds[3] = {0.f, 0.f, 0.f}, dR[3][3];
#pragma unroll
        for (int r = 0; r < 3; r++) {
#pragma unroll
            for (int cc = 0; cc < 3; cc++) {
                const float dm = 2.0f * s[r] * ((R[0][r] * G[0][cc] + R[1][r] * G[1][cc]) + R[2][r] * G[2][cc]);
                ds[r] += dm * R[cc][r];
                dR[cc][r] = s[r] * dm;
            }
        }
        const float dqw = 2.0f * (((-qz * dR[0][1] + qy * dR[0][2]) + (qz * dR[1][0] - qx * dR[1][2])) + (-qy * dR[2][0] + qx * dR[2][1]));
        const float dqx = 2.0f * (((qy * dR[0][1] + qz * dR[0][2]) + (qy * dR[1][0] - 2.0f * qx * dR[1][1] - qw * dR[1][2])) +
                                  (qz * dR[2][0] + qw * dR[2][1] - 2.0f * qx * dR[2][2]));
        const float dqy = 2.0f * (((-2.0f * qy * dR[0][0] + qx * dR[0][1] + qw * dR[0][2]) + (qx * dR[1][0] + qz * dR[1][2])) +
                                  (-qw * dR[2][0] + qz * dR[2][1] - 2.0f * qy * dR[2][2]));
        const float dqz = 2.0f * (((-2.0f * qz * dR[0][0] - qw * dR[0][1] + qx * dR[0][2]) + (qw * dR[1][0] - 2.0f * qz * dR[1][1] + qy * dR[1][2])) +
                                  (qx * dR[2][0] + qy * dR[2][1]));

        gv[0] = dp[0];
        gv[1] = dp[1];
        gv[2] = dp[2];
        gv[4] = ds[0];
        gv[5] = ds[1];
        gv[6] = ds[2];
        gv[7] = AA ? d[5] * comp : d[5];
        gv[8] = dqw;
        gv[9] = dqx;
        gv[10] = dqy;
        gv[11] = dqz;
    }
    if constexpr (CAMERA) {
        __shared__ double s_cam[PB_THREADS / 32][GSB_UBO_WORDS];
        const int lane = threadIdx.x & 31, warp = threadIdx.x >> 5;
#pragma unroll
        for (int j = 0; j < GSB_UBO_WORDS; j++) {
            double a = 0.0;
            if (cam_word_live(j)) {
                a = (double)cam[j];
#pragma unroll
                for (int o = 16; o > 0; o >>= 1) a += __shfl_xor_sync(FULL, a, o);
            }
            if (lane == 0) s_cam[warp][j] = a;
        }
        __syncthreads();
        if (threadIdx.x < GSB_UBO_WORDS) {
            double a = 0.0;
#pragma unroll
            for (int w = 0; w < PB_THREADS / 32; w++) a += s_cam[w][threadIdx.x];
            P.cam_partials[(size_t)blockIdx.x * GSB_UBO_WORDS + threadIdx.x] = a;
        }
    }
}

constexpr int CR_THREADS = 1024;
__global__ void __launch_bounds__(CR_THREADS) k_camera_reduce(const double* __restrict__ partials, uint32_t rows, gsb_uniforms* out) {
    const int lane = threadIdx.x & 31, warp = threadIdx.x >> 5;
    for (int j = warp; j < GSB_UBO_WORDS; j += CR_THREADS / 32) {
        double a = 0.0;
        for (uint32_t r = lane; r < rows; r += 32) a += partials[(size_t)r * GSB_UBO_WORDS + j];
#pragma unroll
        for (int o = 16; o > 0; o >>= 1) a += __shfl_xor_sync(FULL, a, o);
        if (lane == 0) reinterpret_cast<float*>(out)[j] = (float)a;
    }
}

template <int MODE, bool ABSGRAD, bool BG>
cudaError_t launch_blend_det(const BackwardParams& p, float3 bg, cudaStream_t s) {
    constexpr int NACC = BW_NACC + (ABSGRAD ? BW_NABS : 0);
    const size_t smem = (size_t)BW_WARPS * NACC * BW_DET_BATCH * sizeof(float);
    cudaError_t e = cudaFuncSetAttribute(k_blend_backward<MODE, ABSGRAD, true, BG>, cudaFuncAttributeMaxDynamicSharedMemorySize, (int)smem);
    if (e != cudaSuccess) return e;
    k_blend_backward<MODE, ABSGRAD, true, BG><<<p.num_tiles, BW_THREADS, smem, s>>>(bw_params<BG>(p, bg));
    return cudaGetLastError();
}

template <int MODE, bool ABSGRAD>
cudaError_t launch_blend_det(const BackwardParams& p, float3 bg, cudaStream_t s) {
    return has_background(bg) ? launch_blend_det<MODE, ABSGRAD, true>(p, bg, s) : launch_blend_det<MODE, ABSGRAD, false>(p, bg, s);
}

template <bool BG>
void launch_blend_backward(const BackwardParams& p, float3 bg, cudaStream_t s) {
    const bool density = p.density != nullptr;
    if (p.mode == GSB_MODE_EXACT) {
        if (density) k_blend_backward<GSB_MODE_EXACT, true, false, BG><<<p.num_tiles, BW_THREADS, 0, s>>>(bw_params<BG>(p, bg));
        else k_blend_backward<GSB_MODE_EXACT, false, false, BG><<<p.num_tiles, BW_THREADS, 0, s>>>(bw_params<BG>(p, bg));
    } else {
        if (density) k_blend_backward<GSB_MODE_FAST, true, false, BG><<<p.num_tiles, BW_THREADS, 0, s>>>(bw_params<BG>(p, bg));
        else k_blend_backward<GSB_MODE_FAST, false, false, BG><<<p.num_tiles, BW_THREADS, 0, s>>>(bw_params<BG>(p, bg));
    }
}

constexpr int BG_THREADS = 256;
constexpr uint32_t BG_MAX_ROWS = 2048;
__global__ void __launch_bounds__(BG_THREADS) k_background_grad(const uint2* __restrict__ record, const unsigned char* __restrict__ grad_image,
                                                                size_t pitch, uint32_t width, uint32_t height, double* __restrict__ partials) {
    __shared__ double s_w[BG_THREADS / 32][3];
    const int lane = threadIdx.x & 31, warp = threadIdx.x >> 5;
    double a0 = 0.0, a1 = 0.0, a2 = 0.0;
    for (uint32_t y = blockIdx.x; y < height; y += gridDim.x) {
        const uint2* rec = record + (size_t)y * width;
        const float4* g = reinterpret_cast<const float4*>(grad_image + (size_t)y * pitch);
        for (uint32_t x = threadIdx.x; x < width; x += BG_THREADS) {
            const double t = (double)__uint_as_float(__ldg(&rec[x].x));
            const float4 v = __ldg(g + x);
            a0 = __dadd_rn(a0, __dmul_rn(t, (double)v.x));
            a1 = __dadd_rn(a1, __dmul_rn(t, (double)v.y));
            a2 = __dadd_rn(a2, __dmul_rn(t, (double)v.z));
        }
    }
#pragma unroll
    for (int o = 16; o > 0; o >>= 1) {
        a0 += __shfl_xor_sync(FULL, a0, o);
        a1 += __shfl_xor_sync(FULL, a1, o);
        a2 += __shfl_xor_sync(FULL, a2, o);
    }
    if (lane == 0) {
        s_w[warp][0] = a0;
        s_w[warp][1] = a1;
        s_w[warp][2] = a2;
    }
    __syncthreads();
    if (threadIdx.x < 3) {
        double a = 0.0;
#pragma unroll
        for (int w = 0; w < BG_THREADS / 32; w++) a += s_w[w][threadIdx.x];
        partials[(size_t)blockIdx.x * 3 + threadIdx.x] = a;
    }
}

__global__ void __launch_bounds__(96) k_background_reduce(const double* __restrict__ partials, uint32_t rows, float* out) {
    const int lane = threadIdx.x & 31, c = threadIdx.x >> 5;
    double a = 0.0;
    for (uint32_t r = lane; r < rows; r += 32) a += partials[(size_t)r * 3 + c];
#pragma unroll
    for (int o = 16; o > 0; o >>= 1) a += __shfl_xor_sync(FULL, a, o);
    if (lane == 0) out[c] = (float)a;
}

cudaError_t launch_det_sums(const BackwardParams& p, float3 bg, const DetBackward& d, unsigned grid, cudaStream_t s) {
    const bool density = p.density != nullptr;
    cudaError_t e = cudaMemsetAsync(d.sc, 0, sizeof(SortCtl), s);
    if (e != cudaSuccess) return e;
    if ((e = cudaMemsetAsync(d.status, 0, (size_t)d.status_tiles * 256 * sizeof(unsigned long long), s)) != cudaSuccess) return e;
    k_det_prepare<<<grid, PB_THREADS, 0, s>>>(p.vals, p.ctl, d.keys[0], d.pos[0], d.runs);
    if ((e = cudaGetLastError()) != cudaSuccess) return e;
    SortParams sp;
    sp.keys[0] = d.keys[0];
    sp.keys[1] = d.keys[1];
    sp.vals[0] = d.pos[0];
    sp.vals[1] = d.pos[1];
    sp.d_m = &p.ctl->num_instances;
    sp.m_hint = d.m_hint;
    sp.key_bits = d.key_bits;
    sp.status = d.status;
    sp.status_tiles = d.status_tiles;
    sp.epoch_base = 1;
    sp.sc = d.sc;
    sp.num_sms = p.num_sms;
    sp.ranges = d.runs;
    sp.discard_sorted_keys = true;
    uint32_t passes = 0;
    if ((e = launch_sort(sp, &passes, s)) != cudaSuccess) return e;
    if (passes == 0) return cudaErrorInvalidValue;
    if (p.num_tiles) {
        if (p.mode == GSB_MODE_EXACT) e = density ? launch_blend_det<GSB_MODE_EXACT, true>(p, bg, s) : launch_blend_det<GSB_MODE_EXACT, false>(p, bg, s);
        else e = density ? launch_blend_det<GSB_MODE_FAST, true>(p, bg, s) : launch_blend_det<GSB_MODE_FAST, false>(p, bg, s);
        if (e != cudaSuccess) return e;
    }
    const uint32_t* sorted_pos = d.pos[passes & 1];
    if (density) k_det_reduce<true><<<grid, PB_THREADS, 0, s>>>(p, sorted_pos, d.runs);
    else k_det_reduce<false><<<grid, PB_THREADS, 0, s>>>(p, sorted_pos, d.runs);
    return cudaGetLastError();
}

}

cudaError_t launch_backward(const BackwardParams& p, bool antialiased, float3 background, cudaStream_t s, const DetBackward* det) {
    const bool density = p.density != nullptr;
    const unsigned grid = (unsigned)p.num_sms * 4u;
    if (det) {
        cudaError_t e = launch_det_sums(p, background, *det, grid, s);
        if (e != cudaSuccess) return e;
    } else if (p.num_tiles) {
        if (has_background(background)) launch_blend_backward<true>(p, background, s);
        else launch_blend_backward<false>(p, background, s);
        cudaError_t e = cudaGetLastError();
        if (e != cudaSuccess) return e;
    }
    if (density) {
        k_density_accumulate<<<grid, PB_THREADS, 0, s>>>(p);
        cudaError_t e = cudaGetLastError();
        if (e != cudaSuccess) return e;
    }
    if (!p.grad_ubo) {
        if (antialiased) k_preprocess_backward<false, true><<<grid, PB_THREADS, 0, s>>>(p);
        else k_preprocess_backward<false, false><<<grid, PB_THREADS, 0, s>>>(p);
        return cudaGetLastError();
    }
    if (antialiased) k_preprocess_backward<true, true><<<grid, PB_THREADS, 0, s>>>(p);
    else k_preprocess_backward<true, false><<<grid, PB_THREADS, 0, s>>>(p);
    cudaError_t e = cudaGetLastError();
    if (e != cudaSuccess) return e;
    k_camera_reduce<<<1, CR_THREADS, 0, s>>>(p.cam_partials, grid, p.grad_ubo);
    return cudaGetLastError();
}

uint32_t background_grad_rows(uint32_t height) { return std::min(height, BG_MAX_ROWS); }

cudaError_t launch_background_grad(const uint2* record, const float* grad_image, size_t row_pitch_bytes, uint32_t width,
                                   uint32_t height, double* partials, float* out, cudaStream_t s) {
    const uint32_t rows = background_grad_rows(height);
    k_background_grad<<<rows, BG_THREADS, 0, s>>>(record, reinterpret_cast<const unsigned char*>(grad_image), row_pitch_bytes, width,
                                                  height, partials);
    cudaError_t e = cudaGetLastError();
    if (e != cudaSuccess) return e;
    k_background_reduce<<<1, 96, 0, s>>>(partials, rows, out);
    return cudaGetLastError();
}

}
```

3dgs.cpp_b200/csrc/gsb_init.cu:

```cuda
#include <algorithm>

#include "gsb_ctx.cuh"
#include "gsb_geom.cuh"

namespace gsb {
namespace {

constexpr unsigned FULL = 0xffffffffu;
constexpr int BB_THREADS = 256;
constexpr int KNN_THREADS = 256;
constexpr int MAX_LEVELS = 7;

struct BBox {
    float lo[3], hi[3];
    uint32_t nonfinite;
    uint32_t pad;
};

__device__ __forceinline__ float sq_dist(float ax, float ay, float az, float bx, float by, float bz) {
    const float dx = bx - ax, dy = by - ay, dz = bz - az;
    return (dx * dx + dy * dy) + dz * dz;
}

__device__ __forceinline__ uint64_t umin64(uint64_t a, uint64_t b) { return a < b ? a : b; }

__device__ __forceinline__ void insert3(float d, float& b0, float& b1, float& b2) {
    b2 = fminf(b2, fmaxf(b1, d));
    b1 = fminf(b1, fmaxf(b0, d));
    b0 = fminf(b0, d);
}

template <typename T, typename F>
__device__ __forceinline__ T warp_reduce(T v, F op) {
#pragma unroll
    for (int o = 16; o > 0; o >>= 1) v = op(v, __shfl_xor_sync(FULL, v, o));
    return v;
}

__global__ void __launch_bounds__(BB_THREADS) k_init_bbox(const float* __restrict__ xyz, uint64_t n, BBox* __restrict__ partial) {
    __shared__ float s[BB_THREADS / 32][6];
    __shared__ uint32_t s_bad[BB_THREADS / 32];
    float lo[3] = {INFINITY, INFINITY, INFINITY}, hi[3] = {-INFINITY, -INFINITY, -INFINITY};
    uint32_t bad = 0;
    for (uint64_t i = (uint64_t)blockIdx.x * BB_THREADS + threadIdx.x; i < n; i += (uint64_t)gridDim.x * BB_THREADS) {
#pragma unroll
        for (int a = 0; a < 3; a++) {
            const float v = __ldg(xyz + i * 3 + a);
            if (isfinite(v)) {
                lo[a] = fminf(lo[a], v);
                hi[a] = fmaxf(hi[a], v);
            } else {
                bad = 1;
            }
        }
    }
    const int lane = threadIdx.x & 31, warp = threadIdx.x >> 5;
#pragma unroll
    for (int a = 0; a < 3; a++) {
        lo[a] = warp_reduce(lo[a], [](float x, float y) { return fminf(x, y); });
        hi[a] = warp_reduce(hi[a], [](float x, float y) { return fmaxf(x, y); });
    }
    bad = __any_sync(FULL, bad) ? 1u : 0u;
    if (lane == 0) {
        for (int a = 0; a < 3; a++) s[warp][a] = lo[a], s[warp][3 + a] = hi[a];
        s_bad[warp] = bad;
    }
    __syncthreads();
    if (threadIdx.x == 0) {
        BBox b;
        for (int a = 0; a < 3; a++) b.lo[a] = INFINITY, b.hi[a] = -INFINITY;
        b.nonfinite = 0;
        b.pad = 0;
        for (int w = 0; w < BB_THREADS / 32; w++) {
            for (int a = 0; a < 3; a++) b.lo[a] = fminf(b.lo[a], s[w][a]), b.hi[a] = fmaxf(b.hi[a], s[w][3 + a]);
            b.nonfinite |= s_bad[w];
        }
        partial[blockIdx.x] = b;
    }
}

__global__ void k_init_bbox_final(const BBox* __restrict__ partial, int count, BBox* __restrict__ out, uint32_t* d_m, uint32_t n) {
    BBox b = partial[0];
    for (int k = 1; k < count; k++) {
        const BBox p = partial[k];
        for (int a = 0; a < 3; a++) b.lo[a] = fminf(b.lo[a], p.lo[a]), b.hi[a] = fmaxf(b.hi[a], p.hi[a]);
        b.nonfinite |= p.nonfinite;
    }
    *out = b;
    *d_m = n;
}

__device__ __forceinline__ unsigned long long spread21(uint32_t v) {
    unsigned long long x = v & 0x1fffffu;
    x = (x | x << 32) & 0x1f00000000ffffull;
    x = (x | x << 16) & 0x1f0000ff0000ffull;
    x = (x | x << 8) & 0x100f00f00f00f00full;
    x = (x | x << 4) & 0x10c30c30c30c30c3ull;
    x = (x | x << 2) & 0x1249249249249249ull;
    return x;
}

struct MortonGrid {
    float lo[3], scale[3];
};

__global__ void __launch_bounds__(256) k_init_morton(const float* __restrict__ xyz, uint64_t n, const MortonGrid g,
                                                    unsigned long long* __restrict__ keys, uint32_t* __restrict__ vals) {
    for (uint64_t i = (uint64_t)blockIdx.x * blockDim.x + threadIdx.x; i < n; i += (uint64_t)gridDim.x * blockDim.x) {
        unsigned long long code = 0;
#pragma unroll
        for (int a = 0; a < 3; a++) {
            const float c = fminf(fmaxf((__ldg(xyz + i * 3 + a) - g.lo[a]) * g.scale[a], 0.0f), 2097151.0f);
            code |= spread21((uint32_t)c) << a;
        }
        keys[i] = code;
        vals[i] = (uint32_t)i;
    }
}

__global__ void __launch_bounds__(256) k_init_gather(const float* __restrict__ xyz, uint64_t n, const uint32_t* __restrict__ order,
                                                    float4* __restrict__ pts) {
    for (uint64_t i = (uint64_t)blockIdx.x * blockDim.x + threadIdx.x; i < n; i += (uint64_t)gridDim.x * blockDim.x) {
        const uint32_t j = order[i];
        pts[i] = make_float4(__ldg(xyz + (uint64_t)j * 3), __ldg(xyz + (uint64_t)j * 3 + 1), __ldg(xyz + (uint64_t)j * 3 + 2),
                             __uint_as_float(j));
    }
}

__global__ void __launch_bounds__(256) k_init_leaf_boxes(const float4* __restrict__ pts, uint64_t n, uint32_t leaves,
                                                        float4* __restrict__ lo, float4* __restrict__ hi) {
    const uint32_t leaf = (uint32_t)(((uint64_t)blockIdx.x * blockDim.x + threadIdx.x) >> 5);
    if (leaf >= leaves) return;
    const uint64_t i = (uint64_t)leaf * 32 + (threadIdx.x & 31);
    float4 p = i < n ? pts[i] : make_float4(NAN, NAN, NAN, 0.0f);
    const auto mn = [](float x, float y) { return fminf(x, y); };
    const auto mx = [](float x, float y) { return fmaxf(x, y); };
    const float ax = warp_reduce(p.x, mn), ay = warp_reduce(p.y, mn), az = warp_reduce(p.z, mn);
    const float bx = warp_reduce(p.x, mx), by = warp_reduce(p.y, mx), bz = warp_reduce(p.z, mx);
    if ((threadIdx.x & 31) == 0) {
        lo[leaf] = make_float4(ax, ay, az, 0.0f);
        hi[leaf] = make_float4(bx, by, bz, 0.0f);
    }
}

__global__ void __launch_bounds__(256) k_init_node_boxes(const float4* __restrict__ lo_in, const float4* __restrict__ hi_in, uint32_t below,
                                                        uint32_t count, float4* __restrict__ lo, float4* __restrict__ hi) {
    const uint32_t node = (uint32_t)(((uint64_t)blockIdx.x * blockDim.x + threadIdx.x) >> 5);
    if (node >= count) return;
    const uint32_t c = node * 32 + (threadIdx.x & 31);
    const float4 a = c < below ? lo_in[c] : make_float4(NAN, NAN, NAN, 0.0f);
    const float4 b = c < below ? hi_in[c] : make_float4(NAN, NAN, NAN, 0.0f);
    const auto mn = [](float x, float y) { return fminf(x, y); };
    const auto mx = [](float x, float y) { return fmaxf(x, y); };
    const float ax = warp_reduce(a.x, mn), ay = warp_reduce(a.y, mn), az = warp_reduce(a.z, mn);
    const float bx = warp_reduce(b.x, mx), by = warp_reduce(b.y, mx), bz = warp_reduce(b.z, mx);
    if ((threadIdx.x & 31) == 0) {
        lo[node] = make_float4(ax, ay, az, 0.0f);
        hi[node] = make_float4(bx, by, bz, 0.0f);
    }
}

struct Tree {
    const float4* lo;
    const float4* hi;
    uint32_t off[MAX_LEVELS];
    uint32_t cnt[MAX_LEVELS];
    int top;
};

__device__ __forceinline__ uint32_t test_children(const Tree& T, int level, uint32_t first, uint32_t nchild, int lane, bool active,
                                                  float px, float py, float pz, float b2) {
    float4 lo = make_float4(0.f, 0.f, 0.f, 0.f), hi = lo;
    if ((uint32_t)lane < nchild) {
        lo = T.lo[T.off[level] + first + lane];
        hi = T.hi[T.off[level] + first + lane];
    }
    uint32_t mask = 0;
    for (uint32_t c = 0; c < nchild; c++) {
        const float lx = __shfl_sync(FULL, lo.x, c), ly = __shfl_sync(FULL, lo.y, c), lz = __shfl_sync(FULL, lo.z, c);
        const float hx = __shfl_sync(FULL, hi.x, c), hy = __shfl_sync(FULL, hi.y, c), hz = __shfl_sync(FULL, hi.z, c);
        const float bound = sq_dist(px, py, pz, fminf(fmaxf(px, lx), hx), fminf(fmaxf(py, ly), hy), fminf(fmaxf(pz, lz), hz));
        if (__any_sync(FULL, active && bound < b2)) mask |= 1u << c;
    }
    return mask;
}

__global__ void __launch_bounds__(KNN_THREADS) k_init_knn(const float4* __restrict__ pts, uint64_t n, const __grid_constant__ Tree T,
                                                         float* __restrict__ scale) {
    const uint32_t leaf = (uint32_t)(((uint64_t)blockIdx.x * KNN_THREADS + threadIdx.x) >> 5);
    if (leaf >= T.cnt[0]) return;
    const int lane = threadIdx.x & 31;
    const uint64_t i = (uint64_t)leaf * 32 + lane;
    const bool active = i < n;
    const float4 p = active ? pts[i] : make_float4(0.f, 0.f, 0.f, 0.f);
    const uint32_t valid = (uint32_t)umin64(32, n - (uint64_t)leaf * 32);
    float b0 = INFINITY, b1 = INFINITY, b2 = INFINITY;
    for (uint32_t k = 1; k < 32; k++) {
        const uint32_t src = (lane + k) & 31;
        const float qx = __shfl_sync(FULL, p.x, src), qy = __shfl_sync(FULL, p.y, src), qz = __shfl_sync(FULL, p.z, src);
        if (src < valid) insert3(sq_dist(p.x, p.y, p.z, qx, qy, qz), b0, b1, b2);
    }
    if (T.top > 0) {
        int level = T.top;
        uint32_t node = 0;
        uint32_t stack = 0;
        {
            const uint32_t m = test_children(T, level - 1, 0, T.cnt[level - 1], lane, active, p.x, p.y, p.z, b2);
            if (lane == level) stack = m;
        }
        while (true) {
            uint32_t m = __shfl_sync(FULL, stack, level);
            if (m == 0) {
                if (level == T.top) break;
                level++;
                node >>= 5;
                continue;
            }
            const uint32_t a = (leaf >> (5 * (level - 1))) & 31;
            const uint32_t r = __funnelshift_r(m, m, a);
            const uint32_t c = (a + (uint32_t)(__ffs(r) - 1)) & 31;
            m &= ~(1u << c);
            if (lane == level) stack = m;
            const uint32_t child = node * 32 + c;
            if (level == 1) {
                if (child == leaf) continue;
                const uint64_t j = (uint64_t)child * 32 + lane;
                const uint32_t cnt = (uint32_t)umin64(32, n - (uint64_t)child * 32);
                const float4 q = j < n ? pts[j] : make_float4(0.f, 0.f, 0.f, 0.f);
                for (uint32_t k = 0; k < cnt; k++) {
                    const float qx = __shfl_sync(FULL, q.x, k), qy = __shfl_sync(FULL, q.y, k), qz = __shfl_sync(FULL, q.z, k);
                    insert3(sq_dist(p.x, p.y, p.z, qx, qy, qz), b0, b1, b2);
                }
            } else {
                level--;
                node = child;
                const uint32_t nchild = min(32u, T.cnt[level - 1] - child * 32);
                const uint32_t mm = test_children(T, level - 1, child * 32, nchild, lane, active, p.x, p.y, p.z, b2);
                if (lane == level) stack = mm;
            }
        }
    }
    if (!active) return;
    float D;
    if (n >= 4) D = ((b0 + b1) + b2) / 3.0f;
    else if (n == 3) D = (b0 + b1) / 2.0f;
    else if (n == 2) D = b0 / 1.0f;
    else D = 0.0f;
    scale[__float_as_uint(p.w)] = sqrtf(fmaxf(D, 1e-7f));
}

template <bool VEC>
__global__ void __launch_bounds__(256) k_init_records(const float* __restrict__ xyz, const float* __restrict__ rgb, const float* __restrict__ scale,
                                                     uint64_t n, float opacity, float* __restrict__ out) {
    const uint64_t total = n * 15;
    for (uint64_t t = (uint64_t)blockIdx.x * blockDim.x + threadIdx.x; t < total; t += (uint64_t)gridDim.x * blockDim.x) {
        const uint64_t row = t / 15;
        const uint32_t k = (uint32_t)(t - row * 15);
        float4 v = make_float4(0.f, 0.f, 0.f, 0.f);
        if (k == 0) {
            v = make_float4(__ldg(xyz + row * 3), __ldg(xyz + row * 3 + 1), __ldg(xyz + row * 3 + 2), 1.0f);
        } else if (k == 1) {
            const float s = __ldg(scale + row);
            v = make_float4(s, s, s, opacity);
        } else if (k == 2) {
            v.x = 1.0f;
        } else if (k == 3) {
            v.x = (__ldg(rgb + row * 3) - 0.5f) / SH_C0;
            v.y = (__ldg(rgb + row * 3 + 1) - 0.5f) / SH_C0;
            v.z = (__ldg(rgb + row * 3 + 2) - 0.5f) / SH_C0;
        }
        if constexpr (VEC) {
            reinterpret_cast<float4*>(out)[t] = v;
        } else {
            float* o = out + t * 4;
            o[0] = v.x, o[1] = v.y, o[2] = v.z, o[3] = v.w;
        }
    }
}

template <typename T>
T* carve(unsigned char*& at, uint64_t count) {
    T* p = reinterpret_cast<T*>(at);
    at += (count * sizeof(T) + 255) & ~(uint64_t)255;
    return p;
}

unsigned grid_for(uint64_t items, unsigned threads, int num_sms) {
    const uint64_t blocks = (items + threads - 1) / threads;
    return (unsigned)std::max<uint64_t>(1, std::min<uint64_t>(blocks, (uint64_t)num_sms * 16));
}

}
}

using namespace gsb;

extern "C" int gsb_init_from_points(gsb_ctx* ctx, const float* xyz, const float* rgb, uint64_t n, float opacity, float* vertices,
                                    void* stream) {
    if (!ctx) return GSB_ERR_INVALID;
    auto bad = [&](const char* what) { return fail(ctx, GSB_ERR_INVALID, (std::string("gsb_init_from_points: ") + what).c_str()); };
    if (n == 0) return GSB_OK;
    if (!xyz || !rgb || !vertices) return bad("null argument");
    for (const void* p : {(const void*)xyz, (const void*)rgb, (const void*)vertices})
        if (reinterpret_cast<uintptr_t>(p) % 4) return bad("array not aligned to 4 B");
    if (n >= (1ull << 30)) return bad("limited to 2^30 - 1 points");
    if (!(opacity > 0.0f && opacity < 1.0f)) return bad("opacity outside (0, 1) or NaN");
    CK(cudaSetDevice(ctx->device));
    cudaStream_t s = stream_or_own(ctx, stream);

    Tree T{};
    uint64_t nodes = 0;
    {
        uint64_t c = (n + 31) / 32;
        int l = 0;
        while (true) {
            T.off[l] = (uint32_t)nodes;
            T.cnt[l] = (uint32_t)c;
            nodes += c;
            if (c == 1) break;
            c = (c + 31) / 32;
            l++;
        }
        T.top = l;
    }
    const int bb_blocks = (int)grid_for(n, BB_THREADS, ctx->num_sms);
    const uint32_t sort_tiles = (uint32_t)((n + sort_tile_items() - 1) / sort_tile_items());
    uint64_t bytes = 0;
    const auto add = [&](uint64_t b) { bytes += (b + 255) & ~(uint64_t)255; };
    add(sizeof(BBox) * bb_blocks);
    add(sizeof(BBox));
    add(sizeof(SortCtl));
    add(4);
    add((uint64_t)sort_tiles * 256 * 8);
    add(8 * n), add(8 * n), add(4 * n), add(4 * n);
    add(16 * n);
    add(4 * n);
    add(16 * nodes), add(16 * nodes);
    unsigned char* base = nullptr;
    CK(dev_alloc(&base, bytes));
    unsigned char* at = base;
    BBox* partial = carve<BBox>(at, bb_blocks);
    BBox* box = carve<BBox>(at, 1);
    SortCtl* sc = carve<SortCtl>(at, 1);
    uint32_t* d_m = carve<uint32_t>(at, 1);
    unsigned long long* status = carve<unsigned long long>(at, (uint64_t)sort_tiles * 256);
    unsigned long long* keys[2] = {carve<unsigned long long>(at, n), carve<unsigned long long>(at, n)};
    uint32_t* vals[2] = {carve<uint32_t>(at, n), carve<uint32_t>(at, n)};
    float4* pts = carve<float4>(at, n);
    float* scale = carve<float>(at, n);
    float4* lo = carve<float4>(at, nodes);
    float4* hi = carve<float4>(at, nodes);
    T.lo = lo;
    T.hi = hi;

    int rc = GSB_OK;
    cudaError_t e = cudaSuccess;
    const auto run = [&]() -> cudaError_t {
        k_init_bbox<<<bb_blocks, BB_THREADS, 0, s>>>(xyz, n, partial);
        k_init_bbox_final<<<1, 1, 0, s>>>(partial, bb_blocks, box, d_m, (uint32_t)n);
        cudaError_t err = cudaGetLastError();
        if (err != cudaSuccess) return err;
        BBox hb;
        if ((err = cudaMemcpyAsync(&hb, box, sizeof hb, cudaMemcpyDeviceToHost, s)) != cudaSuccess) return err;
        if ((err = cudaStreamSynchronize(s)) != cudaSuccess) return err;
        if (hb.nonfinite) {
            rc = bad("a coordinate is not finite");
            return cudaSuccess;
        }
        MortonGrid g;
        for (int a = 0; a < 3; a++) {
            const double ext = (double)hb.hi[a] - (double)hb.lo[a];
            g.lo[a] = hb.lo[a];
            g.scale[a] = ext > 0.0 ? (float)(2097151.0 / ext) : 0.0f;
        }
        const unsigned grid = grid_for(n, 256, ctx->num_sms);
        k_init_morton<<<grid, 256, 0, s>>>(xyz, n, g, keys[0], vals[0]);
        if ((err = cudaGetLastError()) != cudaSuccess) return err;
        if ((err = cudaMemsetAsync(sc, 0, sizeof(SortCtl), s)) != cudaSuccess) return err;
        if ((err = cudaMemsetAsync(status, 0, (size_t)sort_tiles * 256 * 8, s)) != cudaSuccess) return err;
        SortParams sp;
        sp.keys[0] = keys[0];
        sp.keys[1] = keys[1];
        sp.key_bytes = 8;
        sp.vals[0] = vals[0];
        sp.vals[1] = vals[1];
        sp.d_m = d_m;
        sp.m_hint = (uint32_t)n;
        sp.key_bits = 63;
        sp.status = status;
        sp.status_tiles = sort_tiles;
        sp.epoch_base = 1;
        sp.sc = sc;
        sp.num_sms = ctx->num_sms;
        sp.discard_sorted_keys = true;
        uint32_t passes = 0;
        if ((err = launch_sort(sp, &passes, s)) != cudaSuccess) return err;
        k_init_gather<<<grid, 256, 0, s>>>(xyz, n, vals[passes & 1], pts);
        const uint32_t leaves = T.cnt[0];
        k_init_leaf_boxes<<<(unsigned)(((uint64_t)leaves * 32 + 255) / 256), 256, 0, s>>>(pts, n, leaves, lo, hi);
        if ((err = cudaGetLastError()) != cudaSuccess) return err;
        for (int l = 1; l <= T.top; l++) {
            k_init_node_boxes<<<(unsigned)(((uint64_t)T.cnt[l] * 32 + 255) / 256), 256, 0, s>>>(lo + T.off[l - 1], hi + T.off[l - 1],
                                                                                            T.cnt[l - 1], T.cnt[l], lo + T.off[l],
                                                                                            hi + T.off[l]);
            if ((err = cudaGetLastError()) != cudaSuccess) return err;
        }
        k_init_knn<<<(unsigned)(((uint64_t)leaves * 32 + KNN_THREADS - 1) / KNN_THREADS), KNN_THREADS, 0, s>>>(pts, n, T, scale);
        if ((err = cudaGetLastError()) != cudaSuccess) return err;
        const unsigned rgrid = grid_for(n * 15, 256, ctx->num_sms);
        if (reinterpret_cast<uintptr_t>(vertices) % 16 == 0)
            k_init_records<true><<<rgrid, 256, 0, s>>>(xyz, rgb, scale, n, opacity, vertices);
        else
            k_init_records<false><<<rgrid, 256, 0, s>>>(xyz, rgb, scale, n, opacity, vertices);
        if ((err = cudaGetLastError()) != cudaSuccess) return err;
        return cudaStreamSynchronize(s);
    };
    e = run();
    if (e != cudaSuccess) cudaStreamSynchronize(s);
    cudaFree(base);
    if (e != cudaSuccess) return fail(ctx, e == cudaErrorMemoryAllocation ? GSB_ERR_OOM : GSB_ERR_CUDA, "gsb_init_from_points", e);
    return rc;
}
```

3dgs.cpp_b200/csrc/gsb_internal.cuh:

```cuda
#pragma once
#include <cuda_runtime.h>
#include <stdint.h>

#include <string>

#include "gs_b200.h"

#define GSB_TILE 16
#define GSB_REC_F4 4
#define GSB_MAX_SHARDS 8

namespace gsb {

struct SortCtl {
    uint32_t ticket[8];
    uint32_t hist[8][256];
};

struct Control {
    uint32_t project_ticket;
    uint32_t emit_ticket;
    uint32_t num_visible;
    uint32_t num_instances;
    uint32_t overflow;
    uint32_t overflow_sticky;
    uint32_t epoch;
    uint32_t pad0;
    unsigned long long instances_total;
    unsigned long long blend_consumed;
    unsigned long long candidates_total;
    unsigned long long blend_walked;
    unsigned long long blend_hits;
    unsigned long long blend_staged;
    SortCtl sort_depth;
    SortCtl sort_tile;
    uint32_t route_total[GSB_MAX_SHARDS];
};

struct ProjectParams {
    const float4* pos_op;
    const float4* cov_a;
    const float2* cov_b;
    const float* sh;
    int sh_half;
    uint32_t n;
    uint32_t index_base;
    gsb_uniforms ubo;
    uint32_t tile_row_begin, tile_row_end;
    float4* recs;
    uint32_t* dkeys;
    uint32_t* dvals;
    uint32_t* status;
    Control* ctl;
    uint32_t* dbg_tiles;
    uint4* dbg_aabb;
    int route_world;
    uint32_t band_rows;
    uint32_t* route_status;
    float4* route_dst_recs[GSB_MAX_SHARDS];
    uint32_t* route_dst_dkeys[GSB_MAX_SHARDS];
};

struct EmitParams {
    const uint32_t* sorted_cid;
    uint32_t nv_hint;
    uint32_t tiles_x;
    uint32_t* keys;
    uint32_t* vals;
    uint32_t capacity;
    unsigned long long* status;
    Control* ctl;
    int num_sms;
    const float4* recs;
    int cull;
    uint32_t coarse_shift;
    unsigned long long* dbg_offsets;
};

cudaError_t launch_cov3d(const float* vtx_aos, uint64_t count, uint64_t dst_offset, float4* pos_op,
                         float4* cov_a, float2* cov_b, float* sh, float scale_factor, cudaStream_t s, bool sh_half = false);
cudaError_t launch_project(const ProjectParams& p, bool debug, bool antialiased, cudaStream_t s);
cudaError_t launch_emit(const EmitParams& p, cudaStream_t s);

struct SortParams {
    void* keys[2] = {};
    uint32_t* vals[2] = {};
    int key_bytes = 4;
    const uint32_t* d_m = nullptr;
    uint32_t m_hint = 0;
    uint32_t key_bits = 0;
    unsigned long long* status = nullptr;
    uint32_t status_tiles = 0;
    const uint32_t* d_epoch = nullptr;
    uint32_t epoch_base = 0;
    SortCtl* sc = nullptr;
    int num_sms = 0;
    cudaEvent_t* events = nullptr;
    uint2* ranges = nullptr;
    uint32_t range_key_mask = 0;
    bool discard_sorted_keys = false;
};
cudaError_t launch_sort(const SortParams& p, uint32_t* passes, cudaStream_t s);
uint32_t sort_tile_items();

cudaError_t launch_frame_init(Control* ctl, uint32_t* project_status, uint32_t project_chunks, unsigned long long* emit_status,
                              uint32_t emit_chunks, uint2* ranges, uint32_t num_tiles, cudaStream_t s, uint32_t* route_status = nullptr,
                              uint32_t route_words = 0);
cudaError_t sort_prepare();
cudaError_t launch_ranges_single_tile(const uint32_t* d_m, uint2* ranges, cudaStream_t s);

struct BlendParams {
    const float4* recs;
    const uint32_t* vals;
    const uint32_t* keys;
    const uint2* ranges;
    uint32_t width, height, tiles_x;
    uint32_t coarse_shift, bins_x;
    uint32_t tile_row_begin, tile_row_end;
    void* out;
    uint32_t out_first_row;
    int num_peers;
    void* peer_frames[GSB_MAX_SHARDS];
    size_t row_pitch_bytes;
    int format;
    int mode;
    int stats;
    Control* ctl;
    uint2* record;
    float background[3];
};
cudaError_t launch_blend(const BlendParams& p, cudaStream_t s);

inline bool has_background(const float bg[3]) { return bg[0] != 0.0f || bg[1] != 0.0f || bg[2] != 0.0f; }
inline bool has_background(float3 bg) { return bg.x != 0.0f || bg.y != 0.0f || bg.z != 0.0f; }

struct BackwardParams {
    const float4* recs;
    const uint32_t* vals;
    const uint2* ranges;
    const uint2* record;
    const Control* ctl;
    uint32_t width, height, tiles_x, num_tiles;
    int mode;
    gsb_uniforms ubo;
    const float* vertices;
    const float4* cov_a;
    const float2* cov_b;
    const float* grad_image;
    size_t row_pitch_bytes;
    double* scratch;
    float* grad_vertices;
    int num_sms;
    double* cam_partials;
    gsb_uniforms* grad_ubo;
    double* abs_scratch;
    float* density;
    double* det_slots;
};
#define GSB_UBO_WORDS 40

struct DetBackward {
    uint32_t* keys[2];
    uint32_t* pos[2];
    uint2* runs;
    SortCtl* sc;
    unsigned long long* status;
    uint32_t status_tiles;
    uint32_t m_hint;
    uint32_t key_bits;
};
cudaError_t launch_backward(const BackwardParams& p, bool antialiased, float3 background, cudaStream_t s, const DetBackward* det = nullptr);
uint32_t background_grad_rows(uint32_t height);
cudaError_t launch_background_grad(const uint2* record, const float* grad_image, size_t row_pitch_bytes, uint32_t width,
                                   uint32_t height, double* partials, float* out, cudaStream_t s);

struct AdamParams {
    float4* params;
    float4* exp_avg;
    float4* exp_avg_sq;
    const float4* grad;
    float4* vertices;
    float4* pos_op;
    float4* cov_a;
    float2* cov_b;
    float4* sh;
    uint64_t n;
    const float4* recs;
    const Control* ctl;
    float lr[6];
    float beta1, beta2, eps, bias_correction1, bias_correction2_sqrt;
};
cudaError_t launch_adam(const AdamParams& p, int num_sms, cudaStream_t s);

}
```

3dgs.cpp_b200/csrc/gsb_sort.cu:

```cuda
#include "gsb_internal.cuh"
#include "gsb_tma.cuh"

namespace gsb {

namespace {

#ifndef GSB_SORT_MATCH_ATOMIC
#define GSB_SORT_MATCH_ATOMIC 1
#endif
constexpr int SORT_IPT = 16;
#ifndef GSB_SORT_THREADS
#define GSB_SORT_THREADS 256
#endif
constexpr int SORT_THREADS = GSB_SORT_THREADS;
constexpr int SORT_TILE = SORT_THREADS * SORT_IPT;
constexpr int SORT_WARPS = SORT_THREADS / 32;
constexpr int RADIX = 256;
constexpr unsigned FULL = 0xffffffffu;

#ifndef GSB_HIST_CTAS
#define GSB_HIST_CTAS 3
#endif
constexpr int HIST_THREADS = 512;
constexpr int HIST_IPT = 8;
constexpr int HIST_TILE = HIST_THREADS * HIST_IPT;

constexpr uint32_t LB_AGG = 1u << 30;
constexpr uint32_t LB_PREFIX = 2u << 30;
constexpr uint32_t LB_COUNT = (1u << 30) - 1u;
#ifndef GSB_LB_WINDOW
#define GSB_LB_WINDOW 8
#endif
constexpr int LB_WINDOW = GSB_LB_WINDOW;

__device__ __forceinline__ unsigned long long ld_volatile(const unsigned long long* p) {
    return *reinterpret_cast<const volatile unsigned long long*>(p);
}
__device__ __forceinline__ void st_volatile(unsigned long long* p, unsigned long long v) {
    *reinterpret_cast<volatile unsigned long long*>(p) = v;
}

template <typename KeyT>
__device__ __forceinline__ KeyT key_max();
template <>
__device__ __forceinline__ uint32_t key_max<uint32_t>() {
    return 0xffffffffu;
}
template <>
__device__ __forceinline__ unsigned long long key_max<unsigned long long>() {
    return ~0ull;
}

template <typename KeyT, int P>
__global__ void __launch_bounds__(HIST_THREADS) k_sort_hist(const KeyT* __restrict__ keys, const uint32_t* __restrict__ d_m,
                                                            SortCtl* sc) {
    __shared__ uint32_t s_hist[P][RADIX];
    const int tid = threadIdx.x;
    for (int k = tid; k < P * RADIX; k += HIST_THREADS) (&s_hist[0][0])[k] = 0;
    __syncthreads();
    const uint32_t m = *d_m;
    const uint32_t num_tiles = (m + HIST_TILE - 1) / HIST_TILE;
    for (uint32_t tile = blockIdx.x; tile < num_tiles; tile += gridDim.x) {
        const uint32_t base = tile * HIST_TILE;
        KeyT k[HIST_IPT];
#pragma unroll
        for (int it = 0; it < HIST_IPT; it++) {
            const uint32_t idx = base + it * HIST_THREADS + tid;
            k[it] = idx < m ? __ldg(keys + idx) : key_max<KeyT>();
        }
#pragma unroll
        for (int it = 0; it < HIST_IPT; it++) {
            const uint32_t idx = base + it * HIST_THREADS + tid;
            const bool valid = idx < m;
#pragma unroll
            for (int p = 0; p < P; p++) {
                const uint32_t d = (uint32_t)(k[it] >> (8 * p)) & 255u;
                const uint32_t d0 = __shfl_sync(FULL, d, 0);
                const unsigned same = __ballot_sync(FULL, valid && d == d0);
                if ((threadIdx.x & 31) == 0) {
                    if (same) atomicAdd(&s_hist[p][d0], (uint32_t)__popc(same));
                } else if (valid && d != d0) {
                    atomicAdd(&s_hist[p][d], 1u);
                }
            }
        }
    }
    __syncthreads();
    for (int k = tid; k < P * RADIX; k += HIST_THREADS) {
        const uint32_t c = (&s_hist[0][0])[k];
        if (c) atomicAdd(&sc->hist[0][0] + k, c);
    }
}

template <typename KeyT>
constexpr bool kMatchAtomic = GSB_SORT_MATCH_ATOMIC && sizeof(KeyT) == 4;
template <typename KeyT>
struct PassSmem {
    KeyT keys[2][SORT_TILE];
    uint32_t vals[2][SORT_TILE];
    uint32_t whist[SORT_WARPS][RADIX];
    uint32_t match[kMatchAtomic<KeyT> ? SORT_WARPS : 1][RADIX];
    uint32_t bin_start[RADIX];
    int32_t out_base[RADIX];
    uint32_t gexcl[RADIX];
    uint32_t warp_sums[SORT_WARPS];
    unsigned long long mbar[2];
    uint32_t tile[2];
};
template <typename KeyT>
constexpr int ctas_per_sm() {
    return SORT_THREADS >= 512 ? 1 : 2;
}

__device__ __forceinline__ uint32_t sw(uint32_t d) { return d ^ (d >> 5); }

__device__ __forceinline__ unsigned match_digit8(uint32_t d) {
    unsigned m = FULL;
#pragma unroll
    for (int b = 0; b < 8; b++) {
        const bool bit = (d >> b) & 1u;
        const unsigned vote = __ballot_sync(FULL, bit);
        m &= bit ? vote : ~vote;
    }
    return m;
}

template <int NW>
__device__ __forceinline__ uint32_t block_excl_scan(uint32_t v, uint32_t* warp_sums) {
    const int lane = threadIdx.x & 31, warp = threadIdx.x >> 5;
    uint32_t incl = v;
#pragma unroll
    for (int o = 1; o < 32; o <<= 1) {
        const uint32_t t = __shfl_up_sync(FULL, incl, o);
        if (lane >= o) incl += t;
    }
    if (lane == 31) warp_sums[warp] = incl;
    __syncthreads();
    uint32_t before = 0;
#pragma unroll
    for (int w = 0; w < NW; w++) {
        const uint32_t s = warp_sums[w];
        if (w < warp) before += s;
    }
    __syncthreads();
    return before + incl - v;
}

template <typename KeyT>
__global__ void __launch_bounds__(SORT_THREADS, ctas_per_sm<KeyT>())
    k_onesweep_pass(const KeyT* __restrict__ kin, const uint32_t* __restrict__ vin, KeyT* __restrict__ kout,
                    uint32_t* __restrict__ vout, const uint32_t* __restrict__ d_m, SortCtl* sc, int pass,
                    unsigned long long* status, uint32_t status_tiles, const uint32_t* __restrict__ d_epoch, uint32_t epoch_off,
                    uint2* __restrict__ ranges, uint32_t range_mask) {
    extern __shared__ __align__(128) unsigned char smem_raw[];
    PassSmem<KeyT>& S = *reinterpret_cast<PassSmem<KeyT>*>(smem_raw);
    const int tid = threadIdx.x, lane = tid & 31, warp = tid >> 5;
    const int shift = 8 * pass;
    const uint32_t m = *d_m;
    uint32_t num_tiles = (m + SORT_TILE - 1) / SORT_TILE;
    if (num_tiles > status_tiles) num_tiles = status_tiles;
    const uint32_t epoch = (d_epoch ? *d_epoch : 0u) + epoch_off;
    const unsigned long long epoch_hi = (unsigned long long)epoch << 32;

    auto fetch = [&](int buf) {
        const uint32_t t = atomicAdd(&sc->ticket[pass], 1u);
        S.tile[buf] = t;
        if (t < num_tiles && m - t * SORT_TILE >= (uint32_t)SORT_TILE) {
            fence_proxy_async();
            mbar_expect_tx(&S.mbar[buf], SORT_TILE * (sizeof(KeyT) + 4));
            tma_load(S.keys[buf], kin + (size_t)t * SORT_TILE, SORT_TILE * sizeof(KeyT), &S.mbar[buf]);
            tma_load(S.vals[buf], vin + (size_t)t * SORT_TILE, SORT_TILE * 4, &S.mbar[buf]);
        }
    };

    if (tid == 0) {
        mbar_init(&S.mbar[0], 1);
        mbar_init(&S.mbar[1], 1);
        mbar_fence_init();
    }
    {
        const uint32_t c = tid < RADIX ? sc->hist[pass][tid] : 0u;
        const uint32_t ex = block_excl_scan<SORT_WARPS>(c, S.warp_sums);
        if (tid < RADIX) S.gexcl[tid] = ex;
    }
    if constexpr (kMatchAtomic<KeyT>)
        for (int k = tid; k < SORT_WARPS * RADIX; k += SORT_THREADS) (&S.match[0][0])[k] = 0u;
    if (tid == 0) fetch(0);
    __syncthreads();

    int cur = 0;
    uint32_t parity0 = 0u, parity1 = 0u;
    while (true) {
        const uint32_t tile = S.tile[cur];
        if (tile >= num_tiles) break;
        if (tid == 0) fetch(cur ^ 1);
        const uint32_t tile_base = tile * SORT_TILE;
        const uint32_t valid = min((uint32_t)SORT_TILE, m - tile_base);
        KeyT* sk = S.keys[cur];
        uint32_t* sv = S.vals[cur];

#pragma unroll
        for (int k = 0; k < SORT_WARPS * RADIX / SORT_THREADS; k++) (&S.whist[0][0])[k * SORT_THREADS + tid] = 0;
        if (valid == (uint32_t)SORT_TILE) {
            if (cur == 0) {
                mbar_wait(&S.mbar[0], parity0);
                parity0 ^= 1u;
            } else {
                mbar_wait(&S.mbar[1], parity1);
                parity1 ^= 1u;
            }
        } else {
#pragma unroll 4
            for (int it = 0; it < SORT_IPT; it++) {
                const uint32_t li = it * SORT_THREADS + tid;
                const bool ok = li < valid;
                sk[li] = ok ? __ldg(kin + tile_base + li) : key_max<KeyT>();
                sv[li] = ok ? __ldg(vin + tile_base + li) : 0u;
            }
        }
        __syncthreads();

        const uint32_t wbase = warp * (32 * SORT_IPT) + lane;
        uint16_t rank[SORT_IPT];
        {
            uint32_t dg[SORT_IPT];
#pragma unroll
            for (int it = 0; it < SORT_IPT; it++) dg[it] = sw((uint32_t)(sk[wbase + it * 32] >> shift) & 255u);
            if constexpr (kMatchAtomic<KeyT>) {
#pragma unroll
            for (int it = 0; it < SORT_IPT; it++) {
                volatile uint32_t* mm = &S.match[warp][dg[it]];
                atomicOr(const_cast<uint32_t*>(mm), 1u << lane);
                __syncwarp();
                const unsigned peers = *mm;
                __syncwarp();
                const int leader = __ffs(peers) - 1;
                uint32_t prev = 0;
                if (lane == leader) {
                    *mm = 0u;
                    prev = S.whist[warp][dg[it]];
                    S.whist[warp][dg[it]] = prev + __popc(peers);
                }
                prev = __shfl_sync(FULL, prev, leader);
                rank[it] = (uint16_t)(prev + __popc(peers & ((1u << lane) - 1u)));
                __syncwarp();
            }
            } else {
            unsigned peers[SORT_IPT];
#pragma unroll
            for (int it = 0; it < SORT_IPT; it++) peers[it] = match_digit8(dg[it]);
#pragma unroll
            for (int it = 0; it < SORT_IPT; it++) {
                const int leader = __ffs(peers[it]) - 1;
                uint32_t prev = 0;
                if (lane == leader) {
                    prev = S.whist[warp][dg[it]];
                    S.whist[warp][dg[it]] = prev + __popc(peers[it]);
                }
                prev = __shfl_sync(FULL, prev, leader);
                rank[it] = (uint16_t)(prev + __popc(peers[it] & ((1u << lane) - 1u)));
                __syncwarp();
            }
            }
        }
        __syncthreads();

        uint32_t count = 0;
        if (tid < RADIX) {
#pragma unroll
            for (int w = 0; w < SORT_WARPS; w++) {
                const uint32_t c = S.whist[w][sw(tid)];
                S.whist[w][sw(tid)] = count;
                count += c;
            }
            st_volatile(status + (size_t)tile * RADIX + tid, epoch_hi | (tile == 0 ? LB_PREFIX : LB_AGG) | count);
        }
        const uint32_t bstart = block_excl_scan<SORT_WARPS>(count, S.warp_sums);
        if (tid < RADIX) S.bin_start[sw(tid)] = bstart;
        __syncthreads();

        {
            KeyT key[SORT_IPT];
            uint32_t val[SORT_IPT];
            uint32_t pos[SORT_IPT];
#pragma unroll
            for (int it = 0; it < SORT_IPT; it++) {
                key[it] = sk[wbase + it * 32];
                val[it] = sv[wbase + it * 32];
            }
#pragma unroll
            for (int it = 0; it < SORT_IPT; it++) {
                const uint32_t d = sw((uint32_t)(key[it] >> shift) & 255u);
                pos[it] = S.bin_start[d] + S.whist[warp][d] + rank[it];
            }
            __syncthreads();
#pragma unroll
            for (int it = 0; it < SORT_IPT; it++) {
                sk[pos[it]] = key[it];
                sv[pos[it]] = val[it];
            }
        }

        if (tid < RADIX) {
            uint32_t excl = 0;
            int t = (int)tile - 1;
            bool done = tile == 0;
            while (!done) {
                unsigned long long w[LB_WINDOW];
#pragma unroll
                for (int j = 0; j < LB_WINDOW; j++)
                    w[j] = (t - j >= 0) ? ld_volatile(status + (size_t)(t - j) * RADIX + tid) : (epoch_hi | LB_PREFIX);
#pragma unroll
                for (int j = 0; j < LB_WINDOW; j++) {
                    if (done) break;
                    const uint32_t lo = (uint32_t)w[j];
                    if ((w[j] >> 32) != epoch) break;
                    excl += lo & LB_COUNT;
                    --t;
                    if (lo & LB_PREFIX) done = true;
                }
            }
            if (tile != 0) st_volatile(status + (size_t)tile * RADIX + tid, epoch_hi | LB_PREFIX | (excl + count));
            S.out_base[sw(tid)] = (int32_t)(S.gexcl[tid] + excl) - (int32_t)bstart;
        }
        __syncthreads();

        {
            KeyT k[SORT_IPT];
            uint32_t v[SORT_IPT];
            int32_t g[SORT_IPT];
#pragma unroll
            for (int it = 0; it < SORT_IPT; it++) {
                k[it] = sk[it * SORT_THREADS + tid];
                v[it] = sv[it * SORT_THREADS + tid];
            }
#pragma unroll
            for (int it = 0; it < SORT_IPT; it++)
                g[it] = S.out_base[sw((uint32_t)(k[it] >> shift) & 255u)] + (int32_t)(it * SORT_THREADS + tid);
#pragma unroll
            for (int it = 0; it < SORT_IPT; it++) {
                if ((uint32_t)(it * SORT_THREADS + tid) < valid) {
                    if (kout != nullptr) kout[g[it]] = k[it];
                    vout[g[it]] = v[it];
                }
            }
            if (ranges != nullptr) {
                if constexpr (sizeof(KeyT) == 4) {
#pragma unroll
                    for (int it = 0; it < SORT_IPT; it++) {
                        const uint32_t idx = (uint32_t)(it * SORT_THREADS + tid);
                        if (idx < valid) {
                            const uint32_t key = (uint32_t)k[it] & range_mask;
                            if (idx == 0 || ((uint32_t)sk[idx - 1] & range_mask) != key) atomicMin(&ranges[key].x, (uint32_t)g[it]);
                            if (idx == valid - 1 || ((uint32_t)sk[idx + 1] & range_mask) != key) atomicMin(&ranges[key].y, ~((uint32_t)g[it] + 1u));
                        }
                    }
                }
            }
        }
        __syncthreads();
        cur ^= 1;
    }
}

template <typename KeyT>
cudaError_t launch_hist(const KeyT* keys, const SortParams& p, uint32_t P, uint32_t blocks, cudaStream_t s) {
    switch (P) {
        case 1: k_sort_hist<KeyT, 1><<<blocks, HIST_THREADS, 0, s>>>(keys, p.d_m, p.sc); break;
        case 2: k_sort_hist<KeyT, 2><<<blocks, HIST_THREADS, 0, s>>>(keys, p.d_m, p.sc); break;
        case 3: k_sort_hist<KeyT, 3><<<blocks, HIST_THREADS, 0, s>>>(keys, p.d_m, p.sc); break;
        case 4: k_sort_hist<KeyT, 4><<<blocks, HIST_THREADS, 0, s>>>(keys, p.d_m, p.sc); break;
        default:
            if constexpr (sizeof(KeyT) == 8) {
                switch (P) {
                    case 5: k_sort_hist<KeyT, 5><<<blocks, HIST_THREADS, 0, s>>>(keys, p.d_m, p.sc); break;
                    case 6: k_sort_hist<KeyT, 6><<<blocks, HIST_THREADS, 0, s>>>(keys, p.d_m, p.sc); break;
                    case 7: k_sort_hist<KeyT, 7><<<blocks, HIST_THREADS, 0, s>>>(keys, p.d_m, p.sc); break;
                    default: k_sort_hist<KeyT, 8><<<blocks, HIST_THREADS, 0, s>>>(keys, p.d_m, p.sc); break;
                }
            } else {
                return cudaErrorInvalidValue;
            }
    }
    return cudaGetLastError();
}

template <typename KeyT>
cudaError_t launch_sort_t(const SortParams& p, uint32_t P, cudaStream_t s) {
    const uint32_t hint = p.m_hint ? p.m_hint : 1;
    KeyT* keys[2] = {static_cast<KeyT*>(p.keys[0]), static_cast<KeyT*>(p.keys[1])};
    {
        uint32_t blocks = (hint + HIST_TILE - 1) / HIST_TILE;
        const uint32_t cap = (uint32_t)p.num_sms * GSB_HIST_CTAS;
        if (blocks > cap) blocks = cap;
        if (blocks == 0) blocks = 1;
        cudaError_t e = launch_hist<KeyT>(keys[0], p, P, blocks, s);
        if (e != cudaSuccess) return e;
        if (p.events && (e = cudaEventRecord(p.events[0], s)) != cudaSuccess) return e;
    }
    const size_t smem = sizeof(PassSmem<KeyT>);
    uint32_t blocks = (hint + SORT_TILE - 1) / SORT_TILE;
    const uint32_t cap = (uint32_t)p.num_sms * ctas_per_sm<KeyT>();
    if (blocks > cap) blocks = cap;
    if (blocks == 0) blocks = 1;
    for (uint32_t pass = 0; pass < P; pass++) {
        const int src = pass & 1, dst = src ^ 1;
        KeyT* kout = (pass + 1 == P && p.discard_sorted_keys) ? nullptr : keys[dst];
        k_onesweep_pass<KeyT><<<blocks, SORT_THREADS, smem, s>>>(keys[src], p.vals[src], kout, p.vals[dst], p.d_m, p.sc,
                                                                 (int)pass, p.status, p.status_tiles, p.d_epoch, p.epoch_base + pass,
                                                                 pass + 1 == P ? p.ranges : nullptr, p.range_key_mask ? p.range_key_mask : 0xffffffffu);
        cudaError_t e = cudaGetLastError();
        if (e != cudaSuccess) return e;
        if (p.events && (e = cudaEventRecord(p.events[1 + pass], s)) != cudaSuccess) return e;
    }
    return cudaSuccess;
}

}

uint32_t sort_tile_items() { return SORT_TILE; }

cudaError_t sort_prepare() {
    cudaError_t e = cudaFuncSetAttribute(k_onesweep_pass<uint32_t>, cudaFuncAttributeMaxDynamicSharedMemorySize,
                                         (int)sizeof(PassSmem<uint32_t>));
    if (e != cudaSuccess) return e;
    return cudaFuncSetAttribute(k_onesweep_pass<unsigned long long>, cudaFuncAttributeMaxDynamicSharedMemorySize,
                                (int)sizeof(PassSmem<unsigned long long>));
}

cudaError_t launch_sort(const SortParams& p, uint32_t* passes, cudaStream_t s) {
    const uint32_t P = (p.key_bits + 7) / 8;
    *passes = P;
    if (P == 0) return cudaSuccess;
    if (p.key_bytes == 4 && P <= 4) return launch_sort_t<uint32_t>(p, P, s);
    if (p.key_bytes == 8 && P <= 8) return launch_sort_t<unsigned long long>(p, P, s);
    return cudaErrorInvalidValue;
}

namespace {
__global__ void k_ranges_single_tile(const uint32_t* __restrict__ d_m, uint2* __restrict__ ranges) {
    const uint32_t m = *d_m;
    if (m) ranges[0] = make_uint2(0u, ~m);
}
}

cudaError_t launch_ranges_single_tile(const uint32_t* d_m, uint2* ranges, cudaStream_t s) {
    k_ranges_single_tile<<<1, 1, 0, s>>>(d_m, ranges);
    return cudaGetLastError();
}

}
```

Baseline: 655.2.

## Add configurable wide-digit (up to 11-bit) onesweep radix passes for large tile sorts

Generalises the onesweep radix sort from fixed 8-bit digits to a per-pass digit plan supporting 9–11-bit digits. Wide digits use 512-thread CTAs and 16-bit shared counters, and several shared buffers are unioned to fit the larger histograms. The tile-key sort uses wide digits only when the instance hint is at least 8M and the key fits, aiming to cut the number of scatter passes over large instance arrays. Depth sorting stays at 8 bits, and status and histogram buffers are resized to the largest radix. The cost is larger per-tile status storage, higher shared-memory use and lower occupancy for wide passes, plus more template instantiations.

```diff
diff --git a/3dgs.cpp_b200/csrc/gsb_api.cu b/3dgs.cpp_b200/csrc/gsb_api.cu
--- a/3dgs.cpp_b200/csrc/gsb_api.cu
+++ b/3dgs.cpp_b200/csrc/gsb_api.cu
@@ -56,9 +56,10 @@
 
 int ensure_sort_status(gsb_ctx* ctx, uint64_t items) {
     const uint32_t tiles = (uint32_t)((items + sort_tile_items() - 1) / sort_tile_items());
-    if ((uint64_t)tiles * 256 <= ctx->sort_status.count) return GSB_OK;
+    const uint64_t words = (uint64_t)tiles * sort_status_per_tile();
+    if (words <= ctx->sort_status.count) return GSB_OK;
     ctx->alloc_gen++;
-    return grow_zeroed(ctx, ctx->sort_status, (uint64_t)tiles * 256, "ctx->sort_status");
+    return grow_zeroed(ctx, ctx->sort_status, words, "ctx->sort_status");
 }
 
 int ensure_arena(gsb_ctx* ctx, uint64_t capacity) {
@@ -146,6 +147,10 @@
     return cudaGetLastError();
 }
 
+static uint32_t tile_digit_bits(const FramePlan& fp) {
+    return fp.m_q >= GSB_WIDE_MIN_INSTANCES && bits_for(fp.bins) <= GSB_TILE_DIGIT_BITS ? GSB_TILE_DIGIT_BITS : 8u;
+}
+
 int enqueue_middle(gsb_ctx* ctx, const FramePlan& fp, const Survivors& sv, cudaStream_t stream, bool events) {
     SortParams sa;
     sa.keys[0] = sv.dkeys[0];
@@ -155,8 +160,9 @@
     sa.d_m = &ctx->ctl->num_visible;
     sa.m_hint = fp.nv_q;
     sa.key_bits = 32;
+    sa.digit_bits = GSB_DEPTH_DIGIT_BITS;
     sa.status = ctx->sort_status;
-    sa.status_tiles = (uint32_t)(ctx->sort_status.count / 256);
+    sa.status_tiles = (uint32_t)(ctx->sort_status.count / sort_status_per_tile());
     sa.d_epoch = &ctx->ctl->epoch;
     sa.sc = &ctx->ctl->sort_depth;
     sa.num_sms = ctx->num_sms;
@@ -202,10 +208,11 @@
     sp.d_m = &ctx->ctl->num_instances;
     sp.m_hint = fp.m_q;
     sp.key_bits = bits_for(fp.bins);
+    sp.digit_bits = tile_digit_bits(fp);
     sp.status = ctx->sort_status;
-    sp.status_tiles = (uint32_t)(ctx->sort_status.count / 256);
+    sp.status_tiles = (uint32_t)(ctx->sort_status.count / sort_status_per_tile());
     sp.d_epoch = &ctx->ctl->epoch;
-    sp.epoch_base = 4;
+    sp.epoch_base = fp.depth_passes;
     sp.sc = &ctx->ctl->sort_tile;
     sp.num_sms = ctx->num_sms;
     sp.events = events ? ctx->ev_sort : nullptr;
@@ -295,8 +302,8 @@
         fp.bins_x = fp.tiles_x;
         fp.bins = fp.T;
     }
-    fp.depth_passes = 4;
-    fp.passes = (bits_for(fp.bins) + 7) / 8;
+    fp.depth_passes = sort_pass_count(32, 4, GSB_DEPTH_DIGIT_BITS);
+    fp.passes = sort_pass_count(bits_for(fp.bins), 4, tile_digit_bits(fp));
     fp.fin = (int)(fp.passes & 1);
     if (++ctx->frames_since_epoch_clear >= (1u << 27)) {
         CK(cudaMemsetAsync(ctx->sort_status, 0, ctx->sort_status.count * sizeof(unsigned long long), stream));
@@ -847,7 +854,7 @@
     CK(d.pos[0].grow(cap));
     CK(d.pos[1].grow(cap));
     const uint32_t tiles = (uint32_t)((cap + sort_tile_items() - 1) / sort_tile_items());
-    CK(d.status.grow((uint64_t)std::max<uint32_t>(tiles, 1) * 256));
+    CK(d.status.grow((uint64_t)std::max<uint32_t>(tiles, 1) * sort_status_per_tile()));
     CK(d.sc.grow(1));
     if (n > d.runs.count) CK(d.runs.grow(n));
     return GSB_OK;
@@ -940,7 +947,7 @@
     db.runs = d.runs;
     db.sc = d.sc;
     db.status = d.status;
-    db.status_tiles = (uint32_t)(d.status.count / 256);
+    db.status_tiles = (uint32_t)(d.status.count / sort_status_per_tile());
     db.m_hint = quantise_hint(ctx->m_hint);
     db.key_bits = std::max<uint32_t>(bits_for((uint32_t)n), 1u);
     CK(launch_backward(bp, f.antialiased, bg, s, &db));
@@ -1194,7 +1201,7 @@
     CK(cudaSetDevice(ctx->device));
     cudaStream_t s = stream_or_own(ctx, stream);
     const uint32_t tiles = (uint32_t)((m + sort_tile_items() - 1) / sort_tile_items());
-    const size_t status_bytes = (size_t)tiles * 256 * 8;
+    const size_t status_bytes = (size_t)tiles * sort_status_per_tile() * 8;
     unsigned char* scratch = nullptr;
     CK(dev_alloc(&scratch, status_bytes + sizeof(SortCtl) + 4));
     unsigned long long* status = reinterpret_cast<unsigned long long*>(scratch);
@@ -1214,6 +1221,7 @@
     sp.key_bits = key_bits;
     sp.status = status;
     sp.status_tiles = tiles;
+    sp.digit_bits = key_bytes == 4 ? GSB_SORT_DIGIT_BITS : 8;
     sp.epoch_base = 8;
     sp.sc = sc;
     sp.num_sms = ctx->num_sms;
diff --git a/3dgs.cpp_b200/csrc/gsb_backward.cu b/3dgs.cpp_b200/csrc/gsb_backward.cu
--- a/3dgs.cpp_b200/csrc/gsb_backward.cu
+++ b/3dgs.cpp_b200/csrc/gsb_backward.cu
@@ -624,7 +624,7 @@
     const bool density = p.density != nullptr;
     cudaError_t e = cudaMemsetAsync(d.sc, 0, sizeof(SortCtl), s);
     if (e != cudaSuccess) return e;
-    if ((e = cudaMemsetAsync(d.status, 0, (size_t)d.status_tiles * 256 * sizeof(unsigned long long), s)) != cudaSuccess) return e;
+    if ((e = cudaMemsetAsync(d.status, 0, (size_t)d.status_tiles * sort_status_per_tile() * sizeof(unsigned long long), s)) != cudaSuccess) return e;
     k_det_prepare<<<grid, PB_THREADS, 0, s>>>(p.vals, p.ctl, d.keys[0], d.pos[0], d.runs);
     if ((e = cudaGetLastError()) != cudaSuccess) return e;
     SortParams sp;
diff --git a/3dgs.cpp_b200/csrc/gsb_init.cu b/3dgs.cpp_b200/csrc/gsb_init.cu
--- a/3dgs.cpp_b200/csrc/gsb_init.cu
+++ b/3dgs.cpp_b200/csrc/gsb_init.cu
@@ -331,7 +331,7 @@
     add(sizeof(BBox));
     add(sizeof(SortCtl));
     add(4);
-    add((uint64_t)sort_tiles * 256 * 8);
+    add((uint64_t)sort_tiles * sort_status_per_tile() * 8);
     add(8 * n), add(8 * n), add(4 * n), add(4 * n);
     add(16 * n);
     add(4 * n);
@@ -343,7 +343,7 @@
     BBox* box = carve<BBox>(at, 1);
     SortCtl* sc = carve<SortCtl>(at, 1);
     uint32_t* d_m = carve<uint32_t>(at, 1);
-    unsigned long long* status = carve<unsigned long long>(at, (uint64_t)sort_tiles * 256);
+    unsigned long long* status = carve<unsigned long long>(at, (uint64_t)sort_tiles * sort_status_per_tile());
     unsigned long long* keys[2] = {carve<unsigned long long>(at, n), carve<unsigned long long>(at, n)};
     uint32_t* vals[2] = {carve<uint32_t>(at, n), carve<uint32_t>(at, n)};
     float4* pts = carve<float4>(at, n);
@@ -377,7 +377,7 @@
         k_init_morton<<<grid, 256, 0, s>>>(xyz, n, g, keys[0], vals[0]);
         if ((err = cudaGetLastError()) != cudaSuccess) return err;
         if ((err = cudaMemsetAsync(sc, 0, sizeof(SortCtl), s)) != cudaSuccess) return err;
-        if ((err = cudaMemsetAsync(status, 0, (size_t)sort_tiles * 256 * 8, s)) != cudaSuccess) return err;
+        if ((err = cudaMemsetAsync(status, 0, (size_t)sort_tiles * sort_status_per_tile() * 8, s)) != cudaSuccess) return err;
         SortParams sp;
         sp.keys[0] = keys[0];
         sp.keys[1] = keys[1];
diff --git a/3dgs.cpp_b200/csrc/gsb_internal.cuh b/3dgs.cpp_b200/csrc/gsb_internal.cuh
--- a/3dgs.cpp_b200/csrc/gsb_internal.cuh
+++ b/3dgs.cpp_b200/csrc/gsb_internal.cuh
@@ -12,9 +12,27 @@
 
 namespace gsb {
 
+#ifndef GSB_SORT_DIGIT_BITS
+#define GSB_SORT_DIGIT_BITS 11
+#endif
+#ifndef GSB_DEPTH_DIGIT_BITS
+#define GSB_DEPTH_DIGIT_BITS 8
+#endif
+#ifndef GSB_TILE_DIGIT_BITS
+#define GSB_TILE_DIGIT_BITS GSB_SORT_DIGIT_BITS
+#endif
+#ifndef GSB_WIDE_MIN_INSTANCES
+#define GSB_WIDE_MIN_INSTANCES (1u << 23)
+#endif
+static_assert(GSB_SORT_DIGIT_BITS >= 8 && GSB_SORT_DIGIT_BITS <= 11, "digit widths of 8 to 11 bits");
+constexpr uint32_t SORT_MAX_RADIX = 1u << GSB_SORT_DIGIT_BITS;
+constexpr uint32_t SORT_HIST_WORDS = 8 * 256 > ((32 + GSB_SORT_DIGIT_BITS - 1) / GSB_SORT_DIGIT_BITS) * SORT_MAX_RADIX
+                                         ? 8 * 256
+                                         : ((32 + GSB_SORT_DIGIT_BITS - 1) / GSB_SORT_DIGIT_BITS) * SORT_MAX_RADIX;
+
 struct SortCtl {
     uint32_t ticket[8];
-    uint32_t hist[8][256];
+    uint32_t hist[SORT_HIST_WORDS];
 };
 
 struct Control {
@@ -89,6 +107,7 @@
     const uint32_t* d_m = nullptr;
     uint32_t m_hint = 0;
     uint32_t key_bits = 0;
+    uint32_t digit_bits = 0;
     unsigned long long* status = nullptr;
     uint32_t status_tiles = 0;
     const uint32_t* d_epoch = nullptr;
@@ -101,7 +120,9 @@
     bool discard_sorted_keys = false;
 };
 cudaError_t launch_sort(const SortParams& p, uint32_t* passes, cudaStream_t s);
+uint32_t sort_pass_count(uint32_t key_bits, int key_bytes, uint32_t digit_bits = 0);
 uint32_t sort_tile_items();
+uint32_t sort_status_per_tile();
 
 cudaError_t launch_frame_init(Control* ctl, uint32_t* project_status, uint32_t project_chunks, unsigned long long* emit_status,
                               uint32_t emit_chunks, uint2* ranges, uint32_t num_tiles, cudaStream_t s, uint32_t* route_status = nullptr,
diff --git a/3dgs.cpp_b200/csrc/gsb_sort.cu b/3dgs.cpp_b200/csrc/gsb_sort.cu
--- a/3dgs.cpp_b200/csrc/gsb_sort.cu
+++ b/3dgs.cpp_b200/csrc/gsb_sort.cu
@@ -1,3 +1,6 @@
+#include <algorithm>
+#include <type_traits>
+
 #include "gsb_internal.cuh"
 #include "gsb_tma.cuh"
 
@@ -12,11 +15,19 @@
 #ifndef GSB_SORT_THREADS
 #define GSB_SORT_THREADS 256
 #endif
-constexpr int SORT_THREADS = GSB_SORT_THREADS;
-constexpr int SORT_TILE = SORT_THREADS * SORT_IPT;
-constexpr int SORT_WARPS = SORT_THREADS / 32;
-constexpr int RADIX = 256;
+#ifndef GSB_SORT_WIDE_THREADS
+#define GSB_SORT_WIDE_THREADS 512
+#endif
+constexpr int MAX_BITS = GSB_SORT_DIGIT_BITS;
 constexpr unsigned FULL = 0xffffffffu;
+template <int B>
+struct Layout {
+    static constexpr int THREADS = B > 8 ? GSB_SORT_WIDE_THREADS : GSB_SORT_THREADS;
+    static constexpr int TILE = THREADS * SORT_IPT;
+    static constexpr int WARPS = THREADS / 32;
+    using Ctr = std::conditional_t<(B > 8), uint16_t, uint32_t>;
+    static_assert(sizeof(Ctr) == 4 || TILE < 65536, "16-bit counters need tiles below 65536 pairs");
+};
 
 #ifndef GSB_HIST_CTAS
 #define GSB_HIST_CTAS 3
@@ -51,12 +62,25 @@
     return ~0ull;
 }
 
-template <typename KeyT, int P>
+struct DigitPlan {
+    uint32_t passes;
+    uint32_t table_bits;
+    uint8_t shift[8];
+    uint8_t bits[8];
+};
+
+template <typename KeyT>
+__device__ __forceinline__ uint32_t digit_of(KeyT k, uint32_t shift, uint32_t mask) {
+    return (uint32_t)(k >> shift) & mask;
+}
+
+template <typename KeyT, int P, int B>
 __global__ void __launch_bounds__(HIST_THREADS) k_sort_hist(const KeyT* __restrict__ keys, const uint32_t* __restrict__ d_m,
-                                                            SortCtl* sc) {
-    __shared__ uint32_t s_hist[P][RADIX];
+                                                            SortCtl* sc, DigitPlan dp) {
+    constexpr int R = 1 << B;
+    __shared__ uint32_t s_hist[P][R];
     const int tid = threadIdx.x;
-    for (int k = tid; k < P * RADIX; k += HIST_THREADS) (&s_hist[0][0])[k] = 0;
+    for (int k = tid; k < P * R; k += HIST_THREADS) (&s_hist[0][0])[k] = 0;
     __syncthreads();
     const uint32_t m = *d_m;
     const uint32_t num_tiles = (m + HIST_TILE - 1) / HIST_TILE;
@@ -74,7 +98,7 @@
             const bool valid = idx < m;
 #pragma unroll
             for (int p = 0; p < P; p++) {
-                const uint32_t d = (uint32_t)(k[it] >> (8 * p)) & 255u;
+                const uint32_t d = digit_of(k[it], dp.shift[p], (1u << dp.bits[p]) - 1u);
                 const uint32_t d0 = __shfl_sync(FULL, d, 0);
                 const unsigned same = __ballot_sync(FULL, valid && d == d0);
                 if ((threadIdx.x & 31) == 0) {
@@ -86,38 +110,49 @@
         }
     }
     __syncthreads();
-    for (int k = tid; k < P * RADIX; k += HIST_THREADS) {
+    for (int k = tid; k < P * R; k += HIST_THREADS) {
         const uint32_t c = (&s_hist[0][0])[k];
-        if (c) atomicAdd(&sc->hist[0][0] + k, c);
+        if (c) atomicAdd(&sc->hist[k], c);
     }
 }
 
 template <typename KeyT>
 constexpr bool kMatchAtomic = GSB_SORT_MATCH_ATOMIC && sizeof(KeyT) == 4;
-template <typename KeyT>
+template <typename KeyT, int B>
 struct PassSmem {
+    static constexpr int R = 1 << B;
+    static constexpr int SORT_TILE = Layout<B>::TILE, SORT_WARPS = Layout<B>::WARPS;
+    using Ctr = typename Layout<B>::Ctr;
     KeyT keys[2][SORT_TILE];
     uint32_t vals[2][SORT_TILE];
-    uint32_t whist[SORT_WARPS][RADIX];
-    uint32_t match[kMatchAtomic<KeyT> ? SORT_WARPS : 1][RADIX];
-    uint32_t bin_start[RADIX];
-    int32_t out_base[RADIX];
-    uint32_t gexcl[RADIX];
+    union {
+        Ctr whist[SORT_WARPS][R];
+        int32_t out_base[R];
+    };
+    union {
+        uint32_t match[kMatchAtomic<KeyT> ? SORT_WARPS : 1][256];
+        Ctr bin_start[R];
+    };
+    uint32_t gexcl[R];
     uint32_t warp_sums[SORT_WARPS];
     unsigned long long mbar[2];
     uint32_t tile[2];
 };
-template <typename KeyT>
-constexpr int ctas_per_sm() {
-    return SORT_THREADS >= 512 ? 1 : 2;
-}
-
-__device__ __forceinline__ uint32_t sw(uint32_t d) { return d ^ (d >> 5); }
-
-__device__ __forceinline__ unsigned match_digit8(uint32_t d) {
+template <int B>
+constexpr int ctas_per_sm() { return Layout<B>::THREADS >= 512 ? 1 : 2; }
+
+__device__ __forceinline__ uint32_t sw8(uint32_t d) { return d ^ (d >> 5); }
+template <int B>
+__device__ __forceinline__ uint32_t sw(uint32_t d) {
+    if constexpr (sizeof(typename Layout<B>::Ctr) == 4) return d ^ (d >> 5);
+    else return d ^ ((d >> 6) << 1);
+}
+
+template <int B>
+__device__ __forceinline__ unsigned match_digit(uint32_t d) {
     unsigned m = FULL;
 #pragma unroll
-    for (int b = 0; b < 8; b++) {
+    for (int b = 0; b < B; b++) {
         const bool bit = (d >> b) & 1u;
         const unsigned vote = __ballot_sync(FULL, bit);
         m &= bit ? vote : ~vote;
@@ -146,16 +181,21 @@
     return before + incl - v;
 }
 
-template <typename KeyT>
-__global__ void __launch_bounds__(SORT_THREADS, ctas_per_sm<KeyT>())
+template <typename KeyT, int B>
+__global__ void __launch_bounds__(Layout<B>::THREADS, ctas_per_sm<B>())
     k_onesweep_pass(const KeyT* __restrict__ kin, const uint32_t* __restrict__ vin, KeyT* __restrict__ kout,
-                    uint32_t* __restrict__ vout, const uint32_t* __restrict__ d_m, SortCtl* sc, int pass,
-                    unsigned long long* status, uint32_t status_tiles, const uint32_t* __restrict__ d_epoch, uint32_t epoch_off,
-                    uint2* __restrict__ ranges, uint32_t range_mask) {
+                    uint32_t* __restrict__ vout, const uint32_t* __restrict__ d_m, SortCtl* sc, int pass, uint32_t shift,
+                    uint32_t bits, const uint32_t* __restrict__ ghist, unsigned long long* status, uint32_t status_tiles,
+                    const uint32_t* __restrict__ d_epoch, uint32_t epoch_off, uint2* __restrict__ ranges, uint32_t range_mask) {
+    constexpr int R = 1 << B;
+    constexpr int SORT_THREADS = Layout<B>::THREADS, SORT_TILE = Layout<B>::TILE, SORT_WARPS = Layout<B>::WARPS;
+    using Ctr = typename Layout<B>::Ctr;
+    constexpr int DPT = (R + SORT_THREADS - 1) / SORT_THREADS;
+    constexpr int LBW = LB_WINDOW / DPT >= 2 ? LB_WINDOW / DPT : 2;
     extern __shared__ __align__(128) unsigned char smem_raw[];
-    PassSmem<KeyT>& S = *reinterpret_cast<PassSmem<KeyT>*>(smem_raw);
+    PassSmem<KeyT, B>& S = *reinterpret_cast<PassSmem<KeyT, B>*>(smem_raw);
     const int tid = threadIdx.x, lane = tid & 31, warp = tid >> 5;
-    const int shift = 8 * pass;
+    const uint32_t mask = (1u << bits) - 1u;
     const uint32_t m = *d_m;
     uint32_t num_tiles = (m + SORT_TILE - 1) / SORT_TILE;
     if (num_tiles > status_tiles) num_tiles = status_tiles;
@@ -178,13 +218,28 @@
         mbar_init(&S.mbar[1], 1);
         mbar_fence_init();
     }
+    bool live[DPT];
     {
-        const uint32_t c = tid < RADIX ? sc->hist[pass][tid] : 0u;
-        const uint32_t ex = block_excl_scan<SORT_WARPS>(c, S.warp_sums);
-        if (tid < RADIX) S.gexcl[tid] = ex;
-    }
-    if constexpr (kMatchAtomic<KeyT>)
-        for (int k = tid; k < SORT_WARPS * RADIX; k += SORT_THREADS) (&S.match[0][0])[k] = 0u;
+        uint32_t c[DPT], run = 0;
+#pragma unroll
+        for (int j = 0; j < DPT; j++) {
+            const int d = tid * DPT + j;
+            c[j] = d < R ? ghist[d] : 0u;
+            run += c[j];
+        }
+        uint32_t ex = block_excl_scan<SORT_WARPS>(run, S.warp_sums);
+#pragma unroll
+        for (int j = 0; j < DPT; j++) {
+            const int d = tid * DPT + j;
+            if (d < R) S.gexcl[d] = ex;
+            ex += c[j];
+        }
+#pragma unroll
+        for (int k = 0; k < DPT; k++) {
+            const int d = tid + k * SORT_THREADS;
+            live[k] = d < R && ghist[d] != 0u;
+        }
+    }
     if (tid == 0) fetch(0);
     __syncthreads();
 
@@ -199,8 +254,16 @@
         KeyT* sk = S.keys[cur];
         uint32_t* sv = S.vals[cur];
 
-#pragma unroll
-        for (int k = 0; k < SORT_WARPS * RADIX / SORT_THREADS; k++) (&S.whist[0][0])[k * SORT_THREADS + tid] = 0;
+        static_assert(sizeof(S.whist) % (16 * SORT_THREADS) == 0, "whist is cleared in 16-byte words");
+#pragma unroll
+        for (int k = 0; k < (int)(sizeof(S.whist) / (16 * SORT_THREADS)); k++)
+            reinterpret_cast<uint4*>(&S.whist[0][0])[k * SORT_THREADS + tid] = make_uint4(0u, 0u, 0u, 0u);
+        if constexpr (kMatchAtomic<KeyT>) {
+            static_assert(sizeof(S.match) % (16 * SORT_THREADS) == 0, "match is cleared in 16-byte words");
+#pragma unroll
+            for (int k = 0; k < (int)(sizeof(S.match) / (16 * SORT_THREADS)); k++)
+                reinterpret_cast<uint4*>(&S.match[0][0])[k * SORT_THREADS + tid] = make_uint4(0u, 0u, 0u, 0u);
+        }
         if (valid == (uint32_t)SORT_TILE) {
             if (cur == 0) {
                 mbar_wait(&S.mbar[0], parity0);
@@ -225,21 +288,28 @@
         {
             uint32_t dg[SORT_IPT];
 #pragma unroll
-            for (int it = 0; it < SORT_IPT; it++) dg[it] = sw((uint32_t)(sk[wbase + it * 32] >> shift) & 255u);
+            for (int it = 0; it < SORT_IPT; it++) dg[it] = digit_of(sk[wbase + it * 32], shift, mask);
             if constexpr (kMatchAtomic<KeyT>) {
 #pragma unroll
             for (int it = 0; it < SORT_IPT; it++) {
-                volatile uint32_t* mm = &S.match[warp][dg[it]];
+                volatile uint32_t* mm = &S.match[warp][sw8(dg[it] & 255u)];
                 atomicOr(const_cast<uint32_t*>(mm), 1u << lane);
                 __syncwarp();
-                const unsigned peers = *mm;
+                unsigned peers = *mm;
                 __syncwarp();
-                const int leader = __ffs(peers) - 1;
+                int leader = __ffs(peers) - 1;
+                if (lane == leader) *mm = 0u;
+#pragma unroll
+                for (int b = 8; b < B; b++) {
+                    const bool bit = (dg[it] >> b) & 1u;
+                    const unsigned vote = __ballot_sync(FULL, bit);
+                    peers &= bit ? vote : ~vote;
+                }
+                if constexpr (B > 8) leader = __ffs(peers) - 1;
                 uint32_t prev = 0;
                 if (lane == leader) {
-                    *mm = 0u;
-                    prev = S.whist[warp][dg[it]];
-                    S.whist[warp][dg[it]] = prev + __popc(peers);
+                    prev = S.whist[warp][sw<B>(dg[it])];
+                    S.whist[warp][sw<B>(dg[it])] = (Ctr)(prev + __popc(peers));
                 }
                 prev = __shfl_sync(FULL, prev, leader);
                 rank[it] = (uint16_t)(prev + __popc(peers & ((1u << lane) - 1u)));
@@ -248,14 +318,14 @@
             } else {
             unsigned peers[SORT_IPT];
 #pragma unroll
-            for (int it = 0; it < SORT_IPT; it++) peers[it] = match_digit8(dg[it]);
+            for (int it = 0; it < SORT_IPT; it++) peers[it] = match_digit<B>(dg[it]);
 #pragma unroll
             for (int it = 0; it < SORT_IPT; it++) {
                 const int leader = __ffs(peers[it]) - 1;
                 uint32_t prev = 0;
                 if (lane == leader) {
-                    prev = S.whist[warp][dg[it]];
-                    S.whist[warp][dg[it]] = prev + __popc(peers[it]);
+                    prev = S.whist[warp][sw<B>(dg[it])];
+                    S.whist[warp][sw<B>(dg[it])] = (Ctr)(prev + __popc(peers[it]));
                 }
                 prev = __shfl_sync(FULL, prev, leader);
                 rank[it] = (uint16_t)(prev + __popc(peers[it] & ((1u << lane) - 1u)));
@@ -265,18 +335,41 @@
         }
         __syncthreads();
 
-        uint32_t count = 0;
-        if (tid < RADIX) {
-#pragma unroll
-            for (int w = 0; w < SORT_WARPS; w++) {
-                const uint32_t c = S.whist[w][sw(tid)];
-                S.whist[w][sw(tid)] = count;
-                count += c;
-            }
-            st_volatile(status + (size_t)tile * RADIX + tid, epoch_hi | (tile == 0 ? LB_PREFIX : LB_AGG) | count);
-        }
-        const uint32_t bstart = block_excl_scan<SORT_WARPS>(count, S.warp_sums);
-        if (tid < RADIX) S.bin_start[sw(tid)] = bstart;
+        uint32_t count[DPT];
+#pragma unroll
+        for (int k = 0; k < DPT; k++) {
+            const int d = tid + k * SORT_THREADS;
+            count[k] = 0;
+            if (d < R) {
+#pragma unroll
+                for (int w = 0; w < SORT_WARPS; w++) {
+                    const uint32_t c = S.whist[w][sw<B>(d)];
+                    S.whist[w][sw<B>(d)] = (Ctr)count[k];
+                    count[k] += c;
+                }
+            }
+            if (live[k]) st_volatile(status + (size_t)tile * R + d, epoch_hi | (tile == 0 ? LB_PREFIX : LB_AGG) | count[k]);
+        }
+        if constexpr (DPT == 1) {
+            const uint32_t bstart = block_excl_scan<SORT_WARPS>(count[0], S.warp_sums);
+            if (tid < R) S.bin_start[sw<B>(tid)] = (Ctr)bstart;
+        } else {
+#pragma unroll
+            for (int k = 0; k < DPT; k++) S.bin_start[sw<B>(tid + k * SORT_THREADS)] = (Ctr)count[k];
+            __syncthreads();
+            uint32_t c[DPT], run = 0;
+#pragma unroll
+            for (int j = 0; j < DPT; j++) {
+                c[j] = S.bin_start[sw<B>(tid * DPT + j)];
+                run += c[j];
+            }
+            uint32_t ex = block_excl_scan<SORT_WARPS>(run, S.warp_sums);
+#pragma unroll
+            for (int j = 0; j < DPT; j++) {
+                S.bin_start[sw<B>(tid * DPT + j)] = (Ctr)ex;
+                ex += c[j];
+            }
+        }
         __syncthreads();
 
         {
@@ -290,8 +383,8 @@
             }
 #pragma unroll
             for (int it = 0; it < SORT_IPT; it++) {
-                const uint32_t d = sw((uint32_t)(key[it] >> shift) & 255u);
-                pos[it] = S.bin_start[d] + S.whist[warp][d] + rank[it];
+                const uint32_t d = sw<B>(digit_of(key[it], shift, mask));
+                pos[it] = (uint32_t)S.bin_start[d] + (uint32_t)S.whist[warp][d] + rank[it];
             }
             __syncthreads();
 #pragma unroll
@@ -301,27 +394,49 @@
             }
         }
 
-        if (tid < RADIX) {
-            uint32_t excl = 0;
-            int t = (int)tile - 1;
-            bool done = tile == 0;
-            while (!done) {
-                unsigned long long w[LB_WINDOW];
-#pragma unroll
-                for (int j = 0; j < LB_WINDOW; j++)
-                    w[j] = (t - j >= 0) ? ld_volatile(status + (size_t)(t - j) * RADIX + tid) : (epoch_hi | LB_PREFIX);
-#pragma unroll
-                for (int j = 0; j < LB_WINDOW; j++) {
-                    if (done) break;
-                    const uint32_t lo = (uint32_t)w[j];
-                    if ((w[j] >> 32) != epoch) break;
-                    excl += lo & LB_COUNT;
-                    --t;
-                    if (lo & LB_PREFIX) done = true;
-                }
-            }
-            if (tile != 0) st_volatile(status + (size_t)tile * RADIX + tid, epoch_hi | LB_PREFIX | (excl + count));
-            S.out_base[sw(tid)] = (int32_t)(S.gexcl[tid] + excl) - (int32_t)bstart;
+        {
+            uint32_t excl[DPT];
+            int t[DPT];
+            bool done[DPT];
+#pragma unroll
+            for (int k = 0; k < DPT; k++) {
+                excl[k] = 0;
+                t[k] = (int)tile - 1;
+                done[k] = tile == 0 || !live[k];
+            }
+            while (true) {
+                bool all = true;
+#pragma unroll
+                for (int k = 0; k < DPT; k++) all = all && done[k];
+                if (all) break;
+                unsigned long long w[DPT][LBW];
+#pragma unroll
+                for (int k = 0; k < DPT; k++)
+#pragma unroll
+                    for (int j = 0; j < LBW; j++)
+                        w[k][j] = (!done[k] && t[k] - j >= 0) ? ld_volatile(status + (size_t)(t[k] - j) * R + tid + k * SORT_THREADS)
+                                                              : (epoch_hi | LB_PREFIX);
+#pragma unroll
+                for (int k = 0; k < DPT; k++) {
+#pragma unroll
+                    for (int j = 0; j < LBW; j++) {
+                        if (done[k]) break;
+                        const uint32_t lo = (uint32_t)w[k][j];
+                        if ((w[k][j] >> 32) != epoch) break;
+                        excl[k] += lo & LB_COUNT;
+                        --t[k];
+                        if (lo & LB_PREFIX) done[k] = true;
+                    }
+                }
+            }
+#pragma unroll
+            for (int k = 0; k < DPT; k++) {
+                const int d = tid + k * SORT_THREADS;
+                if (d < R) {
+                    if (tile != 0 && live[k]) st_volatile(status + (size_t)tile * R + d, epoch_hi | LB_PREFIX | (excl[k] + count[k]));
+                    S.out_base[sw<B>(d)] = (int32_t)(S.gexcl[d] + excl[k]) - (int32_t)S.bin_start[sw<B>(d)];
+                }
+            }
         }
         __syncthreads();
 
@@ -336,7 +451,7 @@
             }
 #pragma unroll
             for (int it = 0; it < SORT_IPT; it++)
-                g[it] = S.out_base[sw((uint32_t)(k[it] >> shift) & 255u)] + (int32_t)(it * SORT_THREADS + tid);
+                g[it] = S.out_base[sw<B>(digit_of(k[it], shift, mask))] + (int32_t)(it * SORT_THREADS + tid);
 #pragma unroll
             for (int it = 0; it < SORT_IPT; it++) {
                 if ((uint32_t)(it * SORT_THREADS + tid) < valid) {
@@ -363,30 +478,92 @@
     }
 }
 
+DigitPlan plan_digits(uint32_t key_bits, int key_bytes, uint32_t digit_bits) {
+    DigitPlan dp{};
+    const uint32_t widest = key_bytes == 4 && digit_bits ? std::min<uint32_t>(std::max<uint32_t>(digit_bits, 8u), MAX_BITS) : 8u;
+    dp.passes = (key_bits + widest - 1) / widest;
+    dp.table_bits = 8;
+    uint32_t shift = 0;
+    for (uint32_t p = 0; p < dp.passes; p++) {
+        const uint32_t bits = widest == 8 ? 8u : key_bits / dp.passes + (p < key_bits % dp.passes ? 1u : 0u);
+        dp.shift[p] = (uint8_t)shift;
+        dp.bits[p] = (uint8_t)bits;
+        shift += bits;
+        dp.table_bits = std::max(dp.table_bits, bits);
+    }
+    return dp;
+}
+
+template <typename KeyT, int P>
+void launch_hist_p(const KeyT* keys, const SortParams& p, const DigitPlan& dp, uint32_t blocks, cudaStream_t s) {
+    switch (dp.table_bits) {
+        case 8: k_sort_hist<KeyT, P, 8><<<blocks, HIST_THREADS, 0, s>>>(keys, p.d_m, p.sc, dp); break;
+        case 9: k_sort_hist<KeyT, P, 9><<<blocks, HIST_THREADS, 0, s>>>(keys, p.d_m, p.sc, dp); break;
+        case 10: k_sort_hist<KeyT, P, 10><<<blocks, HIST_THREADS, 0, s>>>(keys, p.d_m, p.sc, dp); break;
+        default: k_sort_hist<KeyT, P, 11><<<blocks, HIST_THREADS, 0, s>>>(keys, p.d_m, p.sc, dp); break;
+    }
+}
+
 template <typename KeyT>
-cudaError_t launch_hist(const KeyT* keys, const SortParams& p, uint32_t P, uint32_t blocks, cudaStream_t s) {
-    switch (P) {
-        case 1: k_sort_hist<KeyT, 1><<<blocks, HIST_THREADS, 0, s>>>(keys, p.d_m, p.sc); break;
-        case 2: k_sort_hist<KeyT, 2><<<blocks, HIST_THREADS, 0, s>>>(keys, p.d_m, p.sc); break;
-        case 3: k_sort_hist<KeyT, 3><<<blocks, HIST_THREADS, 0, s>>>(keys, p.d_m, p.sc); break;
-        case 4: k_sort_hist<KeyT, 4><<<blocks, HIST_THREADS, 0, s>>>(keys, p.d_m, p.sc); break;
-        default:
-            if constexpr (sizeof(KeyT) == 8) {
-                switch (P) {
-                    case 5: k_sort_hist<KeyT, 5><<<blocks, HIST_THREADS, 0, s>>>(keys, p.d_m, p.sc); break;
-                    case 6: k_sort_hist<KeyT, 6><<<blocks, HIST_THREADS, 0, s>>>(keys, p.d_m, p.sc); break;
-                    case 7: k_sort_hist<KeyT, 7><<<blocks, HIST_THREADS, 0, s>>>(keys, p.d_m, p.sc); break;
-                    default: k_sort_hist<KeyT, 8><<<blocks, HIST_THREADS, 0, s>>>(keys, p.d_m, p.sc); break;
-                }
-            } else {
-                return cudaErrorInvalidValue;
-            }
+cudaError_t launch_hist(const KeyT* keys, const SortParams& p, const DigitPlan& dp, uint32_t blocks, cudaStream_t s) {
+    if constexpr (sizeof(KeyT) == 8) {
+        switch (dp.passes) {
+            case 1: k_sort_hist<KeyT, 1, 8><<<blocks, HIST_THREADS, 0, s>>>(keys, p.d_m, p.sc, dp); break;
+            case 2: k_sort_hist<KeyT, 2, 8><<<blocks, HIST_THREADS, 0, s>>>(keys, p.d_m, p.sc, dp); break;
+            case 3: k_sort_hist<KeyT, 3, 8><<<blocks, HIST_THREADS, 0, s>>>(keys, p.d_m, p.sc, dp); break;
+            case 4: k_sort_hist<KeyT, 4, 8><<<blocks, HIST_THREADS, 0, s>>>(keys, p.d_m, p.sc, dp); break;
+            case 5: k_sort_hist<KeyT, 5, 8><<<blocks, HIST_THREADS, 0, s>>>(keys, p.d_m, p.sc, dp); break;
+            case 6: k_sort_hist<KeyT, 6, 8><<<blocks, HIST_THREADS, 0, s>>>(keys, p.d_m, p.sc, dp); break;
+            case 7: k_sort_hist<KeyT, 7, 8><<<blocks, HIST_THREADS, 0, s>>>(keys, p.d_m, p.sc, dp); break;
+            default: k_sort_hist<KeyT, 8, 8><<<blocks, HIST_THREADS, 0, s>>>(keys, p.d_m, p.sc, dp); break;
+        }
+    } else if constexpr (MAX_BITS == 8) {
+        switch (dp.passes) {
+            case 1: k_sort_hist<KeyT, 1, 8><<<blocks, HIST_THREADS, 0, s>>>(keys, p.d_m, p.sc, dp); break;
+            case 2: k_sort_hist<KeyT, 2, 8><<<blocks, HIST_THREADS, 0, s>>>(keys, p.d_m, p.sc, dp); break;
+            case 3: k_sort_hist<KeyT, 3, 8><<<blocks, HIST_THREADS, 0, s>>>(keys, p.d_m, p.sc, dp); break;
+            default: k_sort_hist<KeyT, 4, 8><<<blocks, HIST_THREADS, 0, s>>>(keys, p.d_m, p.sc, dp); break;
+        }
+    } else {
+        switch (dp.passes) {
+            case 1: launch_hist_p<KeyT, 1>(keys, p, dp, blocks, s); break;
+            case 2: launch_hist_p<KeyT, 2>(keys, p, dp, blocks, s); break;
+            case 3: launch_hist_p<KeyT, 3>(keys, p, dp, blocks, s); break;
+            default: k_sort_hist<KeyT, 4, 8><<<blocks, HIST_THREADS, 0, s>>>(keys, p.d_m, p.sc, dp); break;
+        }
     }
     return cudaGetLastError();
 }
 
+template <typename KeyT, int B>
+void launch_pass_b(const KeyT* kin, const uint32_t* vin, KeyT* kout, uint32_t* vout, const SortParams& p, const DigitPlan& dp,
+                   uint32_t pass, uint32_t hint, cudaStream_t s) {
+    uint32_t blocks = (hint + Layout<B>::TILE - 1) / Layout<B>::TILE;
+    const uint32_t cap = (uint32_t)p.num_sms * ctas_per_sm<B>();
+    if (blocks > cap) blocks = cap;
+    if (blocks == 0) blocks = 1;
+    const uint32_t status_tiles = (uint32_t)((uint64_t)p.status_tiles * SORT_MAX_RADIX >> B);
+    k_onesweep_pass<KeyT, B><<<blocks, Layout<B>::THREADS, sizeof(PassSmem<KeyT, B>), s>>>(
+        kin, vin, kout, vout, p.d_m, p.sc, (int)pass, dp.shift[pass], dp.bits[pass], p.sc->hist + (pass << dp.table_bits), p.status,
+        status_tiles, p.d_epoch, p.epoch_base + pass, pass + 1 == dp.passes ? p.ranges : nullptr,
+        p.range_key_mask ? p.range_key_mask : 0xffffffffu);
+}
+
 template <typename KeyT>
-cudaError_t launch_sort_t(const SortParams& p, uint32_t P, cudaStream_t s) {
+void launch_pass(const KeyT* kin, const uint32_t* vin, KeyT* kout, uint32_t* vout, const SortParams& p, const DigitPlan& dp,
+                 uint32_t pass, uint32_t hint, cudaStream_t s) {
+    const uint32_t b = dp.bits[pass];
+    if constexpr (sizeof(KeyT) == 4 && MAX_BITS >= 9)
+        if (b == 9) return launch_pass_b<KeyT, 9>(kin, vin, kout, vout, p, dp, pass, hint, s);
+    if constexpr (sizeof(KeyT) == 4 && MAX_BITS >= 10)
+        if (b == 10) return launch_pass_b<KeyT, 10>(kin, vin, kout, vout, p, dp, pass, hint, s);
+    if constexpr (sizeof(KeyT) == 4 && MAX_BITS >= 11)
+        if (b == 11) return launch_pass_b<KeyT, 11>(kin, vin, kout, vout, p, dp, pass, hint, s);
+    launch_pass_b<KeyT, 8>(kin, vin, kout, vout, p, dp, pass, hint, s);
+}
+
+template <typename KeyT>
+cudaError_t launch_sort_t(const SortParams& p, const DigitPlan& dp, cudaStream_t s) {
     const uint32_t hint = p.m_hint ? p.m_hint : 1;
     KeyT* keys[2] = {static_cast<KeyT*>(p.keys[0]), static_cast<KeyT*>(p.keys[1])};
     {
@@ -394,21 +571,14 @@
         const uint32_t cap = (uint32_t)p.num_sms * GSB_HIST_CTAS;
         if (blocks > cap) blocks = cap;
         if (blocks == 0) blocks = 1;
-        cudaError_t e = launch_hist<KeyT>(keys[0], p, P, blocks, s);
+        cudaError_t e = launch_hist<KeyT>(keys[0], p, dp, blocks, s);
         if (e != cudaSuccess) return e;
         if (p.events && (e = cudaEventRecord(p.events[0], s)) != cudaSuccess) return e;
     }
-    const size_t smem = sizeof(PassSmem<KeyT>);
-    uint32_t blocks = (hint + SORT_TILE - 1) / SORT_TILE;
-    const uint32_t cap = (uint32_t)p.num_sms * ctas_per_sm<KeyT>();
-    if (blocks > cap) blocks = cap;
-    if (blocks == 0) blocks = 1;
-    for (uint32_t pass = 0; pass < P; pass++) {
+    for (uint32_t pass = 0; pass < dp.passes; pass++) {
         const int src = pass & 1, dst = src ^ 1;
-        KeyT* kout = (pass + 1 == P && p.discard_sorted_keys) ? nullptr : keys[dst];
-        k_onesweep_pass<KeyT><<<blocks, SORT_THREADS, smem, s>>>(keys[src], p.vals[src], kout, p.vals[dst], p.d_m, p.sc,
-                                                                 (int)pass, p.status, p.status_tiles, p.d_epoch, p.epoch_base + pass,
-                                                                 pass + 1 == P ? p.ranges : nullptr, p.range_key_mask ? p.range_key_mask : 0xffffffffu);
+        KeyT* kout = (pass + 1 == dp.passes && p.discard_sorted_keys) ? nullptr : keys[dst];
+        launch_pass<KeyT>(keys[src], p.vals[src], kout, p.vals[dst], p, dp, pass, hint, s);
         cudaError_t e = cudaGetLastError();
         if (e != cudaSuccess) return e;
         if (p.events && (e = cudaEventRecord(p.events[1 + pass], s)) != cudaSuccess) return e;
@@ -416,24 +586,43 @@
     return cudaSuccess;
 }
 
-}
-
-uint32_t sort_tile_items() { return SORT_TILE; }
+template <typename KeyT, int B>
+cudaError_t opt_in_smem() {
+    static_assert(sizeof(PassSmem<KeyT, B>) <= 227 * 1024, "an H100 CTA has at most 227 KB of shared memory");
+    cudaError_t e = cudaFuncSetAttribute(k_onesweep_pass<KeyT, B>, cudaFuncAttributePreferredSharedMemoryCarveout, 100);
+    if (e != cudaSuccess) return e;
+    return cudaFuncSetAttribute(k_onesweep_pass<KeyT, B>, cudaFuncAttributeMaxDynamicSharedMemorySize, (int)sizeof(PassSmem<KeyT, B>));
+}
+
+}
+
+uint32_t sort_tile_items() { return Layout<MAX_BITS>::TILE; }
+
+uint32_t sort_status_per_tile() { return SORT_MAX_RADIX; }
+
+uint32_t sort_pass_count(uint32_t key_bits, int key_bytes, uint32_t digit_bits) {
+    return plan_digits(key_bits, key_bytes, digit_bits).passes;
+}
 
 cudaError_t sort_prepare() {
-    cudaError_t e = cudaFuncSetAttribute(k_onesweep_pass<uint32_t>, cudaFuncAttributeMaxDynamicSharedMemorySize,
-                                         (int)sizeof(PassSmem<uint32_t>));
-    if (e != cudaSuccess) return e;
-    return cudaFuncSetAttribute(k_onesweep_pass<unsigned long long>, cudaFuncAttributeMaxDynamicSharedMemorySize,
-                                (int)sizeof(PassSmem<unsigned long long>));
+    cudaError_t e = opt_in_smem<unsigned long long, 8>();
+    if (e == cudaSuccess) e = opt_in_smem<uint32_t, 8>();
+    if constexpr (MAX_BITS >= 9)
+        if (e == cudaSuccess) e = opt_in_smem<uint32_t, 9>();
+    if constexpr (MAX_BITS >= 10)
+        if (e == cudaSuccess) e = opt_in_smem<uint32_t, 10>();
+    if constexpr (MAX_BITS >= 11)
+        if (e == cudaSuccess) e = opt_in_smem<uint32_t, 11>();
+    return e;
 }
 
 cudaError_t launch_sort(const SortParams& p, uint32_t* passes, cudaStream_t s) {
-    const uint32_t P = (p.key_bits + 7) / 8;
-    *passes = P;
-    if (P == 0) return cudaSuccess;
-    if (p.key_bytes == 4 && P <= 4) return launch_sort_t<uint32_t>(p, P, s);
-    if (p.key_bytes == 8 && P <= 8) return launch_sort_t<unsigned long long>(p, P, s);
+    if (p.key_bits > 8u * (uint32_t)p.key_bytes) return cudaErrorInvalidValue;
+    const DigitPlan dp = plan_digits(p.key_bits, p.key_bytes, p.digit_bits);
+    *passes = dp.passes;
+    if (dp.passes == 0) return cudaSuccess;
+    if (p.key_bytes == 4) return launch_sort_t<uint32_t>(p, dp, s);
+    if (p.key_bytes == 8) return launch_sort_t<unsigned long long>(p, dp, s);
     return cudaErrorInvalidValue;
 }
 
```

After: 662.1 (median of 6 runs). 1.1% higher.
